# haotiansun14/rl-rep

Measured on NVIDIA B200. Metric: agent updates/sec, higher is better.
Workload: dtype tf32

## Files before the change

include/rlrep_b200.h:

```cpp
#ifndef RLREP_B200_H_
#define RLREP_B200_H_

#include <stddef.h>
#include <stdint.h>

#ifdef __cplusplus
extern "C" {
#endif

#if defined(__GNUC__)
#define RLREP_EXPORT __attribute__((visibility("default")))
#else
#define RLREP_EXPORT
#endif

#define RLREP_ABI_VERSION 3

RLREP_EXPORT int rlrep_abi_version(void);
RLREP_EXPORT const char* rlrep_last_error(void);


enum { RLREP_ACT_NONE = 0, RLREP_ACT_ELU = 1, RLREP_ACT_RELU = 2, RLREP_ACT_TANH = 3, RLREP_ACT_SIN = 4 };
enum {
  RLREP_DACT_NONE = 0,
// ... 185 lines not shown
RLREP_EXPORT int rlrep_mulv_tensor_read(rlrep_mulv* h, int i, float* out_host);
RLREP_EXPORT int rlrep_mulv_tensor_write(rlrep_mulv* h, int i, const float* in_host);
RLREP_EXPORT int rlrep_mulv_sync_targets(rlrep_mulv* h);
RLREP_EXPORT int rlrep_mulv_update(rlrep_mulv* h, const unsigned char* img, const float* action, const float* reward,
                                   const float* discount, const unsigned char* next_img, const unsigned char* img_step1,
                                   const int* shifts, const float* eps_z, const float* eps_act, const float* noise,
                                   float stddev, float* metrics_host);
RLREP_EXPORT int rlrep_mulv_act_batch(rlrep_mulv* h, const unsigned char* obs, const float* eps_host, float stddev, int n,
                                      float* actions_host);
RLREP_EXPORT int rlrep_mulv_act(rlrep_mulv* h, const unsigned char* obs_host, const float* eps_host, float stddev,
                                float* action_host);
RLREP_EXPORT int rlrep_mulv_update_resident(rlrep_mulv* h, int n_steps, float stddev, float* total_ms);
RLREP_EXPORT int rlrep_mulv_profile_update(rlrep_mulv* h, float stddev, int max_entries, const char** names, float* ms,
                                           double* bytes, double* flops, int* n_entries);
RLREP_EXPORT int rlrep_mulv_last_launches(rlrep_mulv* h, int* launches);

typedef struct rlrep_ldiff rlrep_ldiff;
typedef struct rlrep_ldiff_config {
  int batch_size, action_dim, latent_dim, feature_dim, bn_dim, psi_hidden_dim, psi_hidden_depth, zeta_hidden_dim,
      zeta_hidden_depth, hidden_dim;
  double ae_lr, score_lr, actor_lr, critic_lr, weight_decay;
  float tau, kl_coef, ae_coef, stddev_clip;
  int precision;
} rlrep_ldiff_config;
typedef struct rlrep_ldiff_inputs {
  const unsigned char* frames;
  const unsigned char* next_frames;
  const int* shifts;
  const int* next_shifts;
  const float *action, *reward, *discount;
  const float* eps_post;
  const float *alphabar, *temb, *noise;
  const float* psi_masks;
  const float* zeta_masks;
  const float* eps_act;
  float stddev;
} rlrep_ldiff_inputs;
RLREP_EXPORT int rlrep_ldiff_create(const rlrep_ldiff_config* cfg, void* stream, rlrep_ldiff** out);
RLREP_EXPORT int rlrep_ldiff_destroy(rlrep_ldiff* h);
RLREP_EXPORT int rlrep_ldiff_num_tensors(rlrep_ldiff* h, int* n);
RLREP_EXPORT int rlrep_ldiff_tensor_info(rlrep_ldiff* h, int i, const char** name, float** ptr_dev, int* rows, int* cols);
RLREP_EXPORT int rlrep_ldiff_tensor_read(rlrep_ldiff* h, int i, float* out_host);
RLREP_EXPORT int rlrep_ldiff_tensor_write(rlrep_ldiff* h, int i, const float* in_host);
RLREP_EXPORT int rlrep_ldiff_sync_targets(rlrep_ldiff* h);
RLREP_EXPORT int rlrep_ldiff_update(rlrep_ldiff* h, const rlrep_ldiff_inputs* in, float* metrics_host);
RLREP_EXPORT int rlrep_ldiff_update_resident(rlrep_ldiff* h, int n_steps, float stddev, float* total_ms);
RLREP_EXPORT int rlrep_ldiff_profile_update(rlrep_ldiff* h, float stddev, int max_entries, const char** names, float* ms,
                                            double* bytes, double* flops, int* n_entries);
RLREP_EXPORT int rlrep_ldiff_last_launches(rlrep_ldiff* h, int* launches);

RLREP_EXPORT int rlrep_agent_act_batch(rlrep_agent* agent, const float* states_host, const float* eps_host, int rows,
                                       float* actions_host);
RLREP_EXPORT int rlrep_agent_last_launches(rlrep_agent* agent, int* launches);

#ifdef __cplusplus
}
#endif
#endif
```

rlrep_b200/_lib.py:

```python
from __future__ import annotations

import ctypes as C
from pathlib import Path

_HERE = Path(__file__).resolve().parent
LIB_PATH = _HERE / "librlrep_b200.so"


class RlrepError(RuntimeError):
    pass


class OptimState(C.Structure):
    _fields_ = [("steps", C.c_int), ("t_feature", C.c_longlong), ("t_critic", C.c_longlong), ("t_actor", C.c_longlong),
                ("t_alpha", C.c_longlong), ("log_alpha", C.c_double), ("log_alpha_m", C.c_double),
                ("log_alpha_v", C.c_double)]


class AgentConfig(C.Structure):
    _fields_ = [
        ("alg", C.c_int), ("state_dim", C.c_int), ("action_dim", C.c_int), ("batch_size", C.c_int),
        ("hidden_dim", C.c_int), ("feature_dim", C.c_int), ("actor_hidden_dim", C.c_int), ("feature_steps", C.c_int),
        ("lr_critic", C.c_double), ("lr_feature", C.c_double), ("lr_actor", C.c_double), ("lr_alpha", C.c_double),
        ("discount", C.c_float), ("tau", C.c_float), ("feature_tau", C.c_float), ("alpha", C.c_double),
# ... 91 lines not shown
                                     C.POINTER(C.c_double), C.POINTER(i)],
        "rlrep_gemm_set_debug_buffer": [vp],
        "rlrep_ldiff_create": [vp, vp, C.POINTER(vp)],
        "rlrep_ldiff_destroy": [vp],
        "rlrep_ldiff_num_tensors": [vp, C.POINTER(i)],
        "rlrep_ldiff_tensor_info": [vp, i, C.POINTER(C.c_char_p), C.POINTER(vp), C.POINTER(i), C.POINTER(i)],
        "rlrep_ldiff_tensor_read": [vp, i, vp],
        "rlrep_ldiff_tensor_write": [vp, i, vp],
        "rlrep_ldiff_sync_targets": [vp],
        "rlrep_ldiff_update": [vp, vp, vp],
        "rlrep_ldiff_update_resident": [vp, i, C.c_float, C.POINTER(C.c_float)],
        "rlrep_ldiff_profile_update": [vp, C.c_float, i, C.POINTER(C.c_char_p), C.POINTER(C.c_float),
                                       C.POINTER(C.c_double), C.POINTER(C.c_double), C.POINTER(i)],
        "rlrep_ldiff_last_launches": [vp, C.POINTER(i)],
        "rlrep_mulv_create": [vp, vp, C.POINTER(vp)],
        "rlrep_mulv_destroy": [vp],
        "rlrep_mulv_num_tensors": [vp, C.POINTER(i)],
        "rlrep_mulv_tensor_info": [vp, i, C.POINTER(C.c_char_p), C.POINTER(vp), C.POINTER(i), C.POINTER(i)],
        "rlrep_mulv_tensor_read": [vp, i, vp],
        "rlrep_mulv_tensor_write": [vp, i, vp],
        "rlrep_mulv_sync_targets": [vp],
        "rlrep_mulv_update": [vp, vp, vp, vp, vp, vp, vp, vp, vp, vp, vp, C.c_float, vp],
        "rlrep_mulv_last_launches": [vp, C.POINTER(i)],
        "rlrep_mulv_act": [vp, vp, vp, C.c_float, vp],
        "rlrep_mulv_act_batch": [vp, vp, vp, C.c_float, i, vp],
        "rlrep_mulv_update_resident": [vp, i, C.c_float, C.POINTER(C.c_float)],
        "rlrep_mulv_profile_update": [vp, C.c_float, i, C.POINTER(C.c_char_p), C.POINTER(C.c_float), C.POINTER(C.c_double),
                                      C.POINTER(C.c_double), C.POINTER(i)],
        "rlrep_comm_unique_id": [vp],
        "rlrep_comm_create": [vp, i, i, C.POINTER(vp)],
        "rlrep_comm_destroy": [vp],
        "rlrep_comm_info": [vp, C.POINTER(i), C.POINTER(i), C.POINTER(i), C.POINTER(C.c_longlong)],
        "rlrep_agent_create_sharded": [C.POINTER(AgentConfig), vp, vp, C.POINTER(vp)],
        "rlrep_agent_num_tensors": [vp, C.POINTER(i)],
        "rlrep_agent_tensor_info": [vp, i, C.POINTER(C.c_char_p), C.POINTER(vp), C.POINTER(i), C.POINTER(i)],
        "rlrep_agent_tensor_read": [vp, i, vp],
        "rlrep_agent_tensor_write": [vp, i, vp],
        "rlrep_agent_sync_targets": [vp],
        "rlrep_agent_get_log_alpha": [vp, C.POINTER(C.c_double)],
        "rlrep_agent_set_log_alpha": [vp, C.c_double],
        "rlrep_agent_get_steps": [vp, C.POINTER(i)],
        "rlrep_agent_get_optim_state": [vp, C.POINTER(OptimState)],
        "rlrep_agent_set_optim_state": [vp, C.POINTER(OptimState)],
        "rlrep_agent_train_counts": [vp, C.POINTER(i), C.POINTER(i), C.POINTER(i)],
        "rlrep_agent_train": [vp, vp, vp, i, vp, i, vp, i],
        "rlrep_agent_act": [vp, vp, vp, vp],
        "rlrep_pixring_create": [C.c_longlong, i, i, i, i, C.POINTER(vp)],
        "rlrep_pixring_destroy": [vp],
        "rlrep_pixring_write": [vp, C.c_longlong, i, vp, vp, C.c_float, C.c_float, i],
        "rlrep_pixring_flush": [vp],
        "rlrep_pixring_gather": [vp, vp, i, vp, C.c_float, vp, vp, vp, vp, vp, vp],
        "rlrep_agent_act_batch": [vp, vp, vp, i, vp],
        "rlrep_agent_last_launches": [vp, C.POINTER(i)],
        "rlrep_agent_train_resident": [vp, vp, vp, vp, i, C.POINTER(C.c_float)],
        "rlrep_agent_profile_train": [vp, vp, vp, vp, i, C.POINTER(C.c_char_p), C.POINTER(C.c_float),
                                      C.POINTER(C.c_double), C.POINTER(C.c_double), C.POINTER(i)],
    }
    lib.rlrep_agent_metric_name.argtypes = [vp, i]
    lib.rlrep_agent_metric_name.restype = C.c_char_p
    for name, argtypes in sigs.items():
        fn = getattr(lib, name)
        fn.argtypes = argtypes
        fn.restype = C.c_int


def check(rc: int) -> None:
    if rc != 0:
        msg = load().rlrep_last_error()
        raise RlrepError(msg.decode() if msg else f"rlrep call failed with code {rc}")


def current_stream_ptr() -> int:
    import torch
    return torch.cuda.current_stream().cuda_stream


def make_epilogue(bias=None, r1=None, aux=None, pre_out=None, act="none", dact="none", accumulate=False,
                  scale=1.0) -> Epilogue:
    e = Epilogue()
    e.bias = bias.data_ptr() if bias is not None else None
    if r1 is not None:
        e.r1_u, e.r1_v = r1[0].data_ptr(), r1[1].data_ptr()
    if aux is not None:
        e.aux, e.ld_aux = aux.data_ptr(), aux.stride(0)
    if pre_out is not None:
        e.pre_out, e.ld_pre = pre_out.data_ptr(), pre_out.stride(0)
    e.act, e.dact = ACT[act], DACT[dact]
    e.accumulate = int(accumulate)
    e.scale = scale
    return e


def gemm(A, B, C_out, *, a_mn=False, b_mn=False, path="tc", epi: Epilogue | None = None, A2=None, bn=0, split_k=0,
         ws=None):
    lib = load()
    M = A.shape[1] if a_mn else A.shape[0]
    K = A.shape[0] if a_mn else A.shape[1]
    N = B.shape[1] if b_mn else B.shape[0]
    K1 = K
    if A2 is not None:
        K += A2.shape[1]
    assert (B.shape[0] if b_mn else B.shape[1]) == K
    epi = epi or make_epilogue()
    rc = lib.rlrep_gemm(current_stream_ptr(), 0 if path == "tc" else 1, M, N, K, A.data_ptr(), A.stride(0), int(a_mn),
                        A2.data_ptr() if A2 is not None else None, A2.stride(0) if A2 is not None else 0, K1,
                        B.data_ptr(), B.stride(0), int(b_mn), C_out.data_ptr(), C_out.stride(0), C.byref(epi), bn,
# ... 38 lines not shown
```

rlrep_b200/agents.py:

```python
from __future__ import annotations

import ctypes as C
import math

import numpy as np
import torch

from . import _lib


def _orthogonal(out_f, in_f):
    w = torch.empty(out_f, in_f)
    torch.nn.init.orthogonal_(w)
    return w


def _default_linear(out_f, in_f):
    bound = 1.0 / math.sqrt(in_f)
    return (torch.rand(out_f, in_f) * 2 - 1) * bound, (torch.rand(out_f) * 2 - 1) * bound


class _Handle:

    def __init__(self, cfg: _lib.AgentConfig, comm=None):
# ... 52 lines not shown
        i, _, rows, cols = self.index[name]
        lr, lc = self._logical_shape(name, rows, cols)
        arr = torch.as_tensor(value).detach().cpu().float().reshape(-1)
        if arr.numel() != lr * lc:
            raise ValueError(f"{name}: expected {lr * lc} values, got {arr.numel()}")
        if (lr, lc) != (rows, cols):
            full = torch.zeros(rows, cols)
            full[:lr, :lc] = arr.reshape(lr, lc)
            arr = full.reshape(-1)
        arr = np.ascontiguousarray(arr.numpy())
        _lib.check(self.lib.rlrep_agent_tensor_write(self.h, i, arr.ctypes.data))

    def train(self, ring_handle, idx: np.ndarray, eps) -> np.ndarray:
        if isinstance(eps, torch.Tensor):
            torch.cuda.current_stream(eps.device).synchronize()
            eps_ptr, n_eps = eps.data_ptr(), eps.numel()
        else:
            eps_ptr, n_eps = eps.ctypes.data, eps.size
        _lib.check(self.lib.rlrep_agent_train(self.h, ring_handle, idx.ctypes.data, idx.size, eps_ptr, n_eps,
                                              self._metrics.ctypes.data, self._metrics.size))
        return self._metrics

    @property
    def log_alpha(self) -> float:
        v = C.c_double()
        _lib.check(self.lib.rlrep_agent_get_log_alpha(self.h, C.byref(v)))
        return v.value

    @log_alpha.setter
    def log_alpha(self, v):
        _lib.check(self.lib.rlrep_agent_set_log_alpha(self.h, float(v)))

    @property
    def optim_state(self) -> dict:
        st = _lib.OptimState()
        _lib.check(self.lib.rlrep_agent_get_optim_state(self.h, C.byref(st)))
        return {k: getattr(st, k) for k, _ in _lib.OptimState._fields_}

    @optim_state.setter
    def optim_state(self, d):
        st = _lib.OptimState()
        _lib.check(self.lib.rlrep_agent_get_optim_state(self.h, C.byref(st)))
        for k, _ in _lib.OptimState._fields_:
            if k in d:
                setattr(st, k, type(getattr(st, k))(d[k]))
        _lib.check(self.lib.rlrep_agent_set_optim_state(self.h, C.byref(st)))

    @property
    def last_launches(self) -> int:
        v = C.c_int()
        _lib.check(self.lib.rlrep_agent_last_launches(self.h, C.byref(v)))
        return v.value


class SACAgent:

    alg = "sac"

    def __init__(self, state_dim, action_dim, action_space, lr=3e-4, discount=0.99, target_update_period=2, tau=0.005,
                 alpha=0.1, auto_entropy_tuning=True, hidden_dim=1024, *, precision="tf32", use_cuda_graph=True,
                 noise_device="cpu", **extra):
        if noise_device not in ("cpu", "cuda"):
            raise ValueError("noise_device must be 'cpu' or 'cuda'")
        self.noise_device = noise_device
        self.steps = 0
        self.state_dim, self.action_dim = int(state_dim), int(action_dim)
        self.action_range = [float(action_space.low.min()), float(action_space.high.max())]
        self.discount, self.tau = float(discount), float(tau)
        self.target_update_period = int(target_update_period)
        self.learnable_temperature = bool(auto_entropy_tuning)
        self.target_entropy = -action_dim
        self._lr, self._alpha0, self._hidden = float(lr), float(alpha), int(hidden_dim)
        self._precision, self._use_graph = precision, bool(use_cuda_graph)
        self._extra = extra
        self._h: _Handle | None = None
        self._batch = None
        self._pending_state = self._initial_state()

    def _config(self, batch_size) -> _lib.AgentConfig:
        c = _lib.AgentConfig()
        c.alg = _lib.ALG[self.alg]
        c.state_dim, c.action_dim, c.batch_size = self.state_dim, self.action_dim, int(batch_size)
        c.hidden_dim, c.feature_dim, c.actor_hidden_dim = self._pad(self._hidden), 0, self._pad(self._hidden)
        c.feature_steps = 0
        c.lr_critic = c.lr_actor = c.lr_alpha = self._lr
        c.lr_feature = 0.0
        c.discount, c.tau, c.feature_tau = self.discount, self.tau, 0.0
        c.alpha = self._alpha0
        c.target_update_period = self.target_update_period
        c.auto_entropy_tuning = int(self.learnable_temperature)
        c.use_feature_target = 0
        c.precision = _lib.PRECISION[self._precision]
        c.use_cuda_graph = int(self._use_graph)
        return c

    def _layers(self):
        S, A, H = self.state_dim, self.action_dim, self._hidden
        q = [(f"critic.{h}.{i}", o, n, "orth") for h in ("Q1", "Q2") for i, o, n in ((0, H, S + A), (2, H, H), (4, 1, H))]
        return q + self._actor_layers(H)

    def _actor_layers(self, H):
        S, A = self.state_dim, self.action_dim
        return [("actor.trunk.0", H, S, "orth"), ("actor.trunk.2", H, H, "orth"), ("actor.trunk.4", 2 * A, H, "orth")]

    def _initial_state(self):
        sd = {}
# ... 479 lines not shown
```

rlrep_b200/csrc/agent.cuh:

```cuda
#pragma once
#include <cuda_runtime.h>

#include <cstdint>
#include <cstring>
#include <functional>
#include <memory>
#include <string>
#include <unordered_map>
#include <vector>

#include "common.cuh"
#include "gemm.cuh"
#include "gemm_chain.cuh"
#include "kernels.cuh"

namespace rlrep {

class DeviceArena {
 public:
  DeviceArena() = default;
  DeviceArena(const DeviceArena&) = delete;
  DeviceArena& operator=(const DeviceArena&) = delete;
  ~DeviceArena() { release(); }
  template <typename T>
// ... 159 lines not shown
enum Precision : int { PREC_TF32 = 0, PREC_FP32 = 1 };

class GemmRunner {
 public:
  void init(Precision prec, size_t ws_floats);
  ~GemmRunner();
  void run(const GemmArgs& a, cudaStream_t s);
  bool run_compact(GemmArgs a, int wp, int ho, cudaStream_t s);
  bool compact_supported(GemmArgs a, int wp, int ho);
  void set_sm_share(double share) { sm_share_ = share; }

  bool chains_enabled() const { return prec_ == PREC_TF32; }
  void begin_chain(cudaStream_t s);
  void end_chain();
  bool recording() const { return recording_; }

 private:
  void flush_chain();
  bool recording_ = false;
  cudaStream_t chain_stream_ = nullptr;
  std::vector<GemmArgs> pending_;
  std::vector<std::unique_ptr<GemmChain>> chains_;
  Precision prec_ = PREC_TF32;
  double sm_share_ = 1.0;
  float* ws_ = nullptr;
  size_t ws_floats_ = 0;
  float* kg_ws_ = nullptr;
  size_t kg_ws_floats_ = 0;
  std::unordered_map<std::string, TcGemmPlan> plans_;
};

struct Mat {
  const float* p = nullptr;
  int ld = 0;
};
void linear_fwd(GemmRunner& g, cudaStream_t s, int rows, Mat x, const Linear& l, int act, float* y, int ldy,
                Mat x2 = Mat(), int k1 = 0, float* pre_out = nullptr);
void linear_dgrad(GemmRunner& g, cudaStream_t s, int rows, Mat dy, const Linear& l, int dact, Mat aux, float* dx,
                  int lddx, int col0 = 0, int n_cols = -1);
void linear_wgrad(GemmRunner& g, cudaStream_t s, int rows, Mat dy, Mat x, const Linear& l, Mat x2 = Mat(), int k1 = 0,
                  bool bias_grad = true);
inline ColJob bias_job(int rows, Mat dy, const Linear& l) {
  ColJob j;
  j.X = dy.p; j.ld = dy.ld; j.rows = rows; j.cols = l.out; j.u = nullptr; j.out = l.db;
  return j;
}

class GraphReplay {
 public:
  ~GraphReplay() { reset(); }
  void reset();
  void run(cudaStream_t s, bool enabled, const std::function<void()>& body);
  bool captured() const { return exec_ != nullptr; }

 private:
  int calls_ = 0;
  cudaGraph_t graph_ = nullptr;
  cudaGraphExec_t exec_ = nullptr;
};

struct AgentConfig {
  int alg = 0;
  int state_dim = 0, action_dim = 0, batch = 256;
  int hidden_dim = 256, feature_dim = 256, actor_hidden_dim = 256;
  int k_feat = 0;
  double lr = 3e-4, lr_feat = 1e-4, lr_actor = 1e-4, lr_alpha = 1e-4;
  float discount = 0.99f, tau = 0.005f, feature_tau = 0.005f;
  double alpha0 = 0.1;
  int target_update_period = 2, learn_alpha = 1, use_feature_target = 1;
  int precision = PREC_TF32;
  int use_graph = 1;
  int phi_hidden_dim = 0, phi_hidden_depth = 0, mu_hidden_dim = 0, mu_hidden_depth = 0;
  int nabla_hidden_dim = 0, nabla_hidden_depth = 0, num_noise = 20, num_noises = 1000;
  float sigma_scale = 0.449f;
};

class Agent {
 public:
  virtual ~Agent() = default;
  virtual void train(Ring& ring, const long long* idx_host, int n_idx, const float* eps_host, int n_eps,
                     float* metrics_host, int n_metrics) = 0;
  virtual float train_resident(Ring& ring, const long long* idx_host, const float* eps_host, int n_steps) = 0;
  virtual std::vector<ProfileEntry> profile_train(Ring& ring, const long long* idx_host, const float* eps_host) = 0;
  virtual int idx_per_train() const = 0;
  virtual int eps_per_train() const = 0;
  virtual const std::vector<std::string>& metric_names() const = 0;
  virtual std::vector<ParamGroup*> groups() = 0;
  virtual void act(const float* state_host, const float* eps_host, float* action_host) = 0;
  virtual void act_batch(const float* states_host, const float* eps_host, int rows, float* actions_host) = 0;
  virtual void sync_targets_from_params() = 0;

  AgentConfig cfg;
  cudaStream_t stream = nullptr;
  Control* ctl = nullptr;
  int last_launches = 0;
};

std::unique_ptr<Agent> make_sac_agent(const AgentConfig& cfg, cudaStream_t s);
std::unique_ptr<Agent> make_ctrlsac_agent(const AgentConfig& cfg, cudaStream_t s);
std::unique_ptr<Agent> make_vlsac_agent(const AgentConfig& cfg, cudaStream_t s);
std::unique_ptr<Agent> make_spedersac_agent(const AgentConfig& cfg, cudaStream_t s);
std::unique_ptr<Agent> make_diffsrsac_agent(const AgentConfig& cfg, cudaStream_t s);
class Comm;
std::unique_ptr<Agent> make_ctrlsac_sharded_agent(const AgentConfig& cfg, cudaStream_t s, Comm* comm);

}
```

rlrep_b200/csrc/agent_base.cuh:

```cuda
#pragma once
#include "staging.cuh"

#include "agent.cuh"

namespace rlrep {

class SacBase : public Agent {
 public:
  SacBase(const AgentConfig& c, cudaStream_t s) {
    cfg = c;
    stream = s;
    S_ = c.state_dim;
    A_ = c.action_dim;
    B_ = c.batch;
    AH_ = c.actor_hidden_dim;
    RLREP_CHECK(S_ > 0 && A_ > 0 && B_ > 0, "bad agent dimensions");
  }
  ~SacBase() override {
    for (cudaEvent_t e : events_) cudaEventDestroy(e);
    if (side_) cudaStreamDestroy(side_);
    for (cudaStream_t a : aux_)
      if (a) cudaStreamDestroy(a);
    if (metrics_host_) cudaFreeHost(metrics_host_);
    if (idx_host_) cudaFreeHost(idx_host_);
// ... 29 lines not shown
    std::memcpy(metrics_host, metrics_host_, metric_names().size() * sizeof(float));
  }

  float train_resident(Ring& ring, const long long* idx_host, const float* eps_host, int n_steps) override {
    const int ni = idx_per_train(), ne = eps_per_train();
    RLREP_CHECK(ring.S == S_ && ring.A == A_ && n_steps > 0, "bad arguments");
    bind_ring(ring);
    long long* idx_all = nullptr;
    float* eps_all = nullptr;
    RLREP_CUDA(cudaMalloc(&idx_all, (size_t)n_steps * ni * sizeof(long long)));
    RLREP_CUDA(cudaMalloc(&eps_all, (size_t)n_steps * ne * sizeof(float)));
    RLREP_CUDA(cudaMemcpy(idx_all, idx_host, (size_t)n_steps * ni * sizeof(long long), cudaMemcpyHostToDevice));
    RLREP_CUDA(cudaMemcpy(eps_all, eps_host, (size_t)n_steps * ne * sizeof(float), cudaMemcpyHostToDevice));
    cudaEvent_t e0, e1;
    RLREP_CUDA(cudaEventCreate(&e0));
    RLREP_CUDA(cudaEventCreate(&e1));
    RLREP_CUDA(cudaStreamSynchronize(stream));
    RLREP_CUDA(cudaEventRecord(e0, stream));
    for (int i = 0; i < n_steps; ++i) {
      RLREP_CUDA(cudaMemcpyAsync(idx_dev_, idx_all + (size_t)i * ni, (size_t)ni * sizeof(long long),
                                 cudaMemcpyDeviceToDevice, stream));
      RLREP_CUDA(cudaMemcpyAsync(eps_dev_, eps_all + (size_t)i * ne, (size_t)ne * sizeof(float),
                                 cudaMemcpyDeviceToDevice, stream));
      graph_.run(stream, cfg.use_graph != 0, [&] { update(ring); });
    }
    RLREP_CUDA(cudaEventRecord(e1, stream));
    RLREP_CUDA(cudaEventSynchronize(e1));
    float ms = 0.f;
    RLREP_CUDA(cudaEventElapsedTime(&ms, e0, e1));
    cudaEventDestroy(e0);
    cudaEventDestroy(e1);
    cudaFree(idx_all);
    cudaFree(eps_all);
    return ms;
  }

  std::vector<ProfileEntry> profile_train(Ring& ring, const long long* idx_host, const float* eps_host) override {
    const int ni = idx_per_train(), ne = eps_per_train();
    RLREP_CUDA(cudaStreamSynchronize(stream));
    std::memcpy(idx_host_, idx_host, (size_t)ni * sizeof(long long));
    std::memcpy(eps_host_, eps_host, (size_t)ne * sizeof(float));
    RLREP_CUDA(cudaMemcpyAsync(idx_dev_, idx_host_, (size_t)ni * sizeof(long long), cudaMemcpyHostToDevice, stream));
    RLREP_CUDA(cudaMemcpyAsync(eps_dev_, eps_host_, (size_t)ne * sizeof(float), cudaMemcpyHostToDevice, stream));
    serial_ = true;
    profile_begin(stream);
    try {
      update(ring);
    } catch (...) {
      serial_ = false;
      throw;
    }
    serial_ = false;
    return profile_end(stream);
  }

  void act(const float* state_host, const float* eps_host, float* action_host) override {
    act_batch(state_host, eps_host, 1, action_host);
  }
  void act_batch(const float* states_host, const float* eps_host, int rows, float* actions_host) override {
    RLREP_CHECK(rows >= 0 && states_host && actions_host, "bad arguments");
    const Linear l0 = a0_.view(actor_g_), l1 = a1_.view(actor_g_), l2 = a2_.view(actor_g_);
    const int W = S_ + A_;
    for (int done = 0; done < rows; done += kActRows) {
      const int n = std::min(kActRows, rows - done);
      RLREP_CUDA(cudaStreamSynchronize(stream));
      for (int r = 0; r < n; ++r) {
        float* dst = act_in_host_ + (size_t)r * W;
        std::memcpy(dst, states_host + (size_t)(done + r) * S_, S_ * sizeof(float));
        if (eps_host) std::memcpy(dst + S_, eps_host + (size_t)(done + r) * A_, A_ * sizeof(float));
      }
      launch_actor_act(act_in_dev_, n, S_, A_, AH_, l0.W, l0.ld, l0.b, l1.W, l1.ld, l1.b, l2.W, l2.ld, l2.b,
                       eps_host != nullptr, act_out_dev_, stream);
      RLREP_CUDA(cudaStreamSynchronize(stream));
      std::memcpy(actions_host + (size_t)done * A_, act_out_host_, (size_t)n * A_ * sizeof(float));
    }
  }

 protected:
  void bind_ring(const Ring& ring) {
    if (ring_bound_ != ring.generation) {
      graph_.reset();
      ring_bound_ = ring.generation;
    }
  }
  virtual void update(Ring& ring) = 0;

  cudaStream_t side() {
    if (serial_) return stream;
    if (side_ == nullptr) RLREP_CUDA(cudaStreamCreateWithFlags(&side_, cudaStreamNonBlocking));
    return side_;
  }
  cudaEvent_t next_event() {
    if (ev_next_ == events_.size()) {
      cudaEvent_t e;
      RLREP_CUDA(cudaEventCreateWithFlags(&e, cudaEventDisableTiming));
      events_.push_back(e);
    }
    return events_[ev_next_++];
  }
  void fork() {
    gemm_.set_sm_share(dual_share_);
    if (serial_) return;
    cudaEvent_t e = next_event();
    RLREP_CUDA(cudaEventRecord(e, stream));
    RLREP_CUDA(cudaStreamWaitEvent(side(), e, 0));
  }
// ... 48 lines not shown
    arena_.want(&bh2_, (size_t)B_ * AH_);
    arena_.want(&bhead_, (size_t)B_ * round_up32(2 * A_));
    arena_.want(&logp_, B_);
    arena_.want(&dhead_, (size_t)B_ * LDH_);
    arena_.want(&dah2_, (size_t)B_ * AH_);
    arena_.want(&dah1_, (size_t)B_ * AH_);
    LDSA_ = round_up32(S_ + A_);
    arena_.want(&dsa_, (size_t)B_ * LDSA_);
    arena_.want(&cat_next_, (size_t)B_ * LDSA_);
    arena_.want(&cat_pi_, (size_t)B_ * LDSA_);
    arena_.want(&dlogp_, 4);
    RLREP_CUDA(cudaMallocHost(&metrics_host_, kNumMetrics * sizeof(float)));
    RLREP_CUDA(cudaMallocHost(&idx_host_, (size_t)(n_idx > 0 ? n_idx : 1) * sizeof(long long)));
    RLREP_CUDA(cudaMallocHost(&eps_host_, (size_t)(n_eps > 0 ? n_eps : 1) * sizeof(float)));
    RLREP_CUDA(cudaHostAlloc(&act_in_host_, (size_t)kActRows * (S_ + A_) * sizeof(float), cudaHostAllocMapped));
    RLREP_CUDA(cudaHostAlloc(&act_out_host_, (size_t)kActRows * A_ * sizeof(float), cudaHostAllocMapped));
    std::memset(act_in_host_, 0, (size_t)kActRows * (S_ + A_) * sizeof(float));
    RLREP_CUDA(cudaHostGetDevicePointer(&act_in_dev_, act_in_host_, 0));
    RLREP_CUDA(cudaHostGetDevicePointer(&act_out_dev_, act_out_host_, 0));
  }

  void finish_setup(size_t gemm_ws_floats) {
    arena_.commit();
    gemm_.init(static_cast<Precision>(cfg.precision), gemm_ws_floats);
    Control h;
    std::memset(&h, 0, sizeof(h));
    h.log_alpha = std::log(cfg.alpha0);
    h.alpha = (float)cfg.alpha0;
    RLREP_CUDA(cudaMemcpyAsync(ctl, &h, sizeof(h), cudaMemcpyHostToDevice, stream));
    RLREP_CUDA(cudaStreamSynchronize(stream));
  }

  Mat actor_forward_cat(Mat obs, const float* eps, float* cat_buf, float* logp_out, cudaStream_t s = nullptr, int set = 0) {
    if (s == nullptr) s = stream;
    const Linear l0 = a0_.view(actor_g_), l1 = a1_.view(actor_g_), l2 = a2_.view(actor_g_);
    float* h1 = set == 0 ? ah1_ : bh1_;
    float* h2 = set == 0 ? ah2_ : bh2_;
    float* hd = set == 0 ? head_ : bhead_;
    linear_fwd(gemm_, s, B_, obs, l0, ACT_ELU, h1, AH_);
    linear_fwd(gemm_, s, B_, Mat{h1, AH_}, l1, ACT_ELU, h2, AH_);
    linear_fwd(gemm_, s, B_, Mat{h2, AH_}, l2, ACT_NONE, hd, LDH_);
    launch_actor_sample(hd, LDH_, B_, A_, eps, cat_buf + S_, LDSA_, logp_out, s, obs.p, obs.ld, S_);
    return Mat{cat_buf, LDSA_};
  }
  void actor_trunk(Mat obs, int set, cudaStream_t s) {
    const Linear l0 = a0_.view(actor_g_), l1 = a1_.view(actor_g_), l2 = a2_.view(actor_g_);
    float* h1 = set == 0 ? ah1_ : bh1_;
    float* h2 = set == 0 ? ah2_ : bh2_;
    float* hd = set == 0 ? head_ : bhead_;
    linear_fwd(gemm_, s, B_, obs, l0, ACT_ELU, h1, AH_);
    linear_fwd(gemm_, s, B_, Mat{h1, AH_}, l1, ACT_ELU, h2, AH_);
    linear_fwd(gemm_, s, B_, Mat{h2, AH_}, l2, ACT_NONE, hd, LDH_);
  }
  Mat actor_sample_cat(Mat obs, const float* eps, float* cat_buf, float* logp_out, int set, cudaStream_t s) {
    launch_actor_sample(set == 0 ? head_ : bhead_, LDH_, B_, A_, eps, cat_buf + S_, LDSA_, logp_out, s, obs.p, obs.ld, S_);
    return Mat{cat_buf, LDSA_};
  }
  void actor_backward_chained(Mat obs, const float* eps) {
    const Linear l0 = a0_.view(actor_g_), l1 = a1_.view(actor_g_), l2 = a2_.view(actor_g_);
    launch_actor_sample_bwd(head_, LDH_, B_, A_, eps, dsa_ + S_, LDSA_, dlogp_, dhead_, LDH_, stream);
    gemm_.begin_chain(stream);
    linear_wgrad(gemm_, stream, B_, Mat{dhead_, LDH_}, Mat{ah2_, AH_}, l2, Mat(), 0, false);
    linear_dgrad(gemm_, stream, B_, Mat{dhead_, LDH_}, l2, DACT_ELU_OUT, Mat{ah2_, AH_}, dah2_, AH_);
    linear_wgrad(gemm_, stream, B_, Mat{dah2_, AH_}, Mat{ah1_, AH_}, l1, Mat(), 0, false);
    linear_dgrad(gemm_, stream, B_, Mat{dah2_, AH_}, l1, DACT_ELU_OUT, Mat{ah1_, AH_}, dah1_, AH_);
    linear_wgrad(gemm_, stream, B_, Mat{dah1_, AH_}, obs, l0, Mat(), 0, false);
    gemm_.end_chain();
    const ColJob jobs[3] = {bias_job(B_, Mat{dhead_, LDH_}, l2), bias_job(B_, Mat{dah2_, AH_}, l1),
                            bias_job(B_, Mat{dah1_, AH_}, l0)};
    launch_colreduce_multi(jobs, 3, stream);
  }
  struct ActionGradDst {
    float* dx;
    int ld, col0, n_cols;
  };
  ActionGradDst action_grad_dst(const Linear& first) const {
    if (cfg.precision == PREC_TF32 && first.ld == LDSA_ && B_ >= 64) return {dsa_, LDSA_, 0, LDSA_};
    return {dsa_ + S_, LDSA_, S_, A_};
  }
  void dgrad_to_action(Mat dy, const Linear& first) {
    const ActionGradDst d = action_grad_dst(first);
    linear_dgrad(gemm_, stream, B_, dy, first, DACT_NONE, Mat(), d.dx, d.ld, d.col0, d.n_cols);
  }
  void actor_backward(Mat obs, const float* eps) {
    const Linear l0 = a0_.view(actor_g_), l1 = a1_.view(actor_g_), l2 = a2_.view(actor_g_);
    cudaStream_t w = aux(1);
    launch_actor_sample_bwd(head_, LDH_, B_, A_, eps, dsa_ + S_, LDSA_, dlogp_, dhead_, LDH_, stream);
    wait_for(w, mark(stream));
    linear_wgrad(gemm_, w, B_, Mat{dhead_, LDH_}, Mat{ah2_, AH_}, l2, Mat(), 0, false);
    linear_dgrad(gemm_, stream, B_, Mat{dhead_, LDH_}, l2, DACT_ELU_OUT, Mat{ah2_, AH_}, dah2_, AH_);
    wait_for(w, mark(stream));
    linear_wgrad(gemm_, w, B_, Mat{dah2_, AH_}, Mat{ah1_, AH_}, l1, Mat(), 0, false);
    linear_dgrad(gemm_, stream, B_, Mat{dah2_, AH_}, l1, DACT_ELU_OUT, Mat{ah1_, AH_}, dah1_, AH_);
    linear_wgrad(gemm_, stream, B_, Mat{dah1_, AH_}, obs, l0, Mat(), 0, false);
    wait_for(w, mark(stream));
    {
      const ColJob jobs[3] = {bias_job(B_, Mat{dhead_, LDH_}, l2), bias_job(B_, Mat{dah2_, AH_}, l1),
                              bias_job(B_, Mat{dah1_, AH_}, l0)};
      launch_colreduce_multi(jobs, 3, w);
    }
    join_aux(1, stream);
  }
  void actor_adam() {
    launch_adam_polyak(actor_g_.p, actor_g_.g, actor_g_.m, actor_g_.v, actor_g_.n, &ctl->actor, nullptr, 0, 0.f,
                       nullptr, stream);
  }
  TickParams base_tick() const {
    TickParams t;
    t.k_feat = cfg.k_feat;
// ... 39 lines not shown
```

rlrep_b200/csrc/agent_ctrlsac.cu:

```cuda
#include "agent_base.cuh"

namespace rlrep {

namespace {

class CtrlSacAgent final : public SacBase {
 public:
  CtrlSacAgent(const AgentConfig& c, cudaStream_t s) : SacBase(c, s) {
    H_ = c.hidden_dim;
    D_ = c.feature_dim;
    K_ = c.k_feat;
    RLREP_CHECK(K_ >= 1 && K_ <= kMaxFeatureSteps, "extra_feature_steps out of range");
    const RecordLayout probe_layout = RecordLayout::of(S_, A_);
    off_r_ = probe_layout.off_r;
    off_d_ = probe_layout.off_d;
    off_s2_ = probe_layout.off_s2;
    plan_common(K_ * B_, 2 * B_ * A_, probe_layout.R);

    feat_g_.name = "feature";
    p1_ = add_linear(feat_g_, "phi.l1", H_, S_ + A_);
    p2_ = add_linear(feat_g_, "phi.l2", H_, H_);
    p3_ = add_linear(feat_g_, "phi.l3", D_, H_);
    feat_g_.n_target = feat_g_.n;
    feat_g_.target_prefix_from = "phi.";
// ... 161 lines not shown
      GemmArgs a;
      a.M = B_; a.N = D_; a.K = B_;
      a.A = logits_; a.lda = B_; a.a_mn = true;
      a.B = zphi_; a.ldb = D_; a.b_mn = true;
      a.C = dzmu_; a.ldc = D_;
      a.epi.dact = DACT_TANH_OUT; a.epi.aux = zmu_; a.epi.ld_aux = D_;
      gemm_.run(a, s1);
    }
    wait_for(w1, mark(s1));
    gemm_.set_sm_share(wshare);
    linear_wgrad(gemm_, w1, B_, Mat{dzmu_, D_}, Mat{g2_, H_}, n3, Mat(), 0, false);
    gemm_.set_sm_share(share);
    linear_dgrad(gemm_, s1, B_, Mat{dzmu_, D_}, n3, DACT_ELU_OUT, Mat{g2_, H_}, dg2_, H_);
    wait_for(w1, mark(s1));
    gemm_.set_sm_share(wshare);
    linear_wgrad(gemm_, w1, B_, Mat{dg2_, H_}, Mat{g1_, H_}, n2, Mat(), 0, false);
    gemm_.set_sm_share(share);
    linear_dgrad(gemm_, s1, B_, Mat{dg2_, H_}, n2, DACT_ELU_OUT, Mat{g1_, H_}, dg1_, H_);
    linear_wgrad(gemm_, s1, B_, Mat{dg1_, H_}, s2(), n1, Mat(), 0, false);
    wait_for(w1, mark(s1));
    {
      ColJob jobs[3] = {bias_job(B_, Mat{dzmu_, D_}, n3), bias_job(B_, Mat{dg2_, H_}, n2),
                        bias_job(B_, Mat{dg1_, H_}, n1)};
      launch_colreduce_multi(jobs, 3, w1);
    }
    join_aux(0, s0);
    join_aux(1, s0);
    join();
    launch_adam_polyak(feat_g_.p, feat_g_.g, feat_g_.m, feat_g_.v, feat_g_.n, &ctl->feat[k],
                       cfg.use_feature_target ? feat_g_.target : nullptr, feat_g_.n_target, cfg.feature_tau, nullptr,
                       s0);
  }

  void feature_step_chained(int k, Ring& ring) {
    const Linear l1 = p1_.view(feat_g_), l2 = p2_.view(feat_g_), l3 = p3_.view(feat_g_);
    const Linear n1 = m1_.view(feat_g_), n2 = m2_.view(feat_g_), n3 = m3_.view(feat_g_);
    const Linear th = th_.view(feat_g_);
    const float inv_b = 1.f / (float)B_;
    cudaStream_t s0 = stream;
    launch_gather(ring.data, R_ / 4, idx_dev_ + (size_t)k * B_, B_, batch_, s0);
    gemm_.begin_chain(s0);
    phi_forward(s0, sa(), Mat(), 0, zphi_, h1_, h2_);
    linear_fwd(gemm_, s0, B_, s2(), n1, ACT_ELU, g1_, H_);
    linear_fwd(gemm_, s0, B_, Mat{g1_, H_}, n2, ACT_ELU, g2_, H_);
    linear_fwd(gemm_, s0, B_, Mat{g2_, H_}, n3, ACT_TANH, zmu_, D_);
    {
      GemmArgs a;
      a.M = B_; a.N = B_; a.K = D_;
      a.A = zphi_; a.lda = D_;
      a.B = zmu_; a.ldb = D_;
      a.C = logits_; a.ldc = B_;
      gemm_.run(a, s0);
    }
    gemm_.end_chain();
    launch_contrastive_head(logits_, B_, B_, B_, 0, inv_b, zphi_, D_, D_, th.W, th.b, reward(), R_, loss_rows_, rpred_, drp_,
                            metrics_dev_ + 0, head_ctr_, s0);
    gemm_.begin_chain(s0);
    {
      GemmArgs a;
      a.M = B_; a.N = D_; a.K = B_;
      a.A = logits_; a.lda = B_;
      a.B = zmu_; a.ldb = D_; a.b_mn = true;
      a.C = dzphi_; a.ldc = D_;
      a.epi.r1_u = drp_; a.epi.r1_v = th.W;
      gemm_.run(a, s0);
    }
    {
      GemmArgs a;
      a.M = B_; a.N = D_; a.K = B_;
      a.A = logits_; a.lda = B_; a.a_mn = true;
      a.B = zphi_; a.ldb = D_; a.b_mn = true;
      a.C = dzmu_; a.ldc = D_;
      a.epi.dact = DACT_TANH_OUT; a.epi.aux = zmu_; a.epi.ld_aux = D_;
      gemm_.run(a, s0);
    }
    linear_dgrad(gemm_, s0, B_, Mat{dzphi_, D_}, l3, DACT_ELU_OUT, Mat{h2_, H_}, dh2_, H_);
    linear_dgrad(gemm_, s0, B_, Mat{dzmu_, D_}, n3, DACT_ELU_OUT, Mat{g2_, H_}, dg2_, H_);
    linear_wgrad(gemm_, s0, B_, Mat{dzphi_, D_}, Mat{h2_, H_}, l3, Mat(), 0, false);
    linear_wgrad(gemm_, s0, B_, Mat{dzmu_, D_}, Mat{g2_, H_}, n3, Mat(), 0, false);
    linear_dgrad(gemm_, s0, B_, Mat{dh2_, H_}, l2, DACT_ELU_OUT, Mat{h1_, H_}, dh1_, H_);
    linear_dgrad(gemm_, s0, B_, Mat{dg2_, H_}, n2, DACT_ELU_OUT, Mat{g1_, H_}, dg1_, H_);
    linear_wgrad(gemm_, s0, B_, Mat{dh2_, H_}, Mat{h1_, H_}, l2, Mat(), 0, false);
    linear_wgrad(gemm_, s0, B_, Mat{dg2_, H_}, Mat{g1_, H_}, n2, Mat(), 0, false);
    linear_wgrad(gemm_, s0, B_, Mat{dh1_, H_}, sa(), l1, Mat(), 0, false);
    linear_wgrad(gemm_, s0, B_, Mat{dg1_, H_}, s2(), n1, Mat(), 0, false);
    gemm_.end_chain();
    {
      ColJob jobs[8] = {bias_job(B_, Mat{dzphi_, D_}, l3), bias_job(B_, Mat{dh2_, H_}, l2),
                        bias_job(B_, Mat{dh1_, H_}, l1), ColJob{zphi_, drp_, th.dW, D_, B_, D_},
                        ColJob{drp_, nullptr, th.db, 1, B_, 1},
                        bias_job(B_, Mat{dzmu_, D_}, n3), bias_job(B_, Mat{dg2_, H_}, n2),
                        bias_job(B_, Mat{dg1_, H_}, n1)};
      launch_colreduce_multi(jobs, 8, s0);
    }
    launch_adam_polyak(feat_g_.p, feat_g_.g, feat_g_.m, feat_g_.v, feat_g_.n, &ctl->feat[k],
                       cfg.use_feature_target ? feat_g_.target : nullptr, feat_g_.n_target, cfg.feature_tau, nullptr,
                       s0);
  }

  void critic_step_chained() {
    cudaStream_t s0 = stream;
    const float* eps_next = eps_dev_;
    const float* eps_pi = eps_dev_ + (size_t)B_ * A_;
    const Linear l14t = c14_.view(crit_g_, true), l14 = c14_.view(crit_g_), l2 = c2_.view(crit_g_), l5 = c5_.view(crit_g_);
    const Linear l2t = c2_.view(crit_g_, true), l5t = c5_.view(crit_g_, true);
    gemm_.begin_chain(s0);
    actor_trunk(s2(), 1, s0);
    actor_trunk(Mat{batch_, R_}, 0, s0);
    gemm_.end_chain();
    const Mat s2a = actor_sample_cat(s2(), eps_next, cat_next_, logp2_, 1, s0);
    const Mat spi = actor_sample_cat(Mat{batch_, R_}, eps_pi, cat_pi_, logp_, 0, s0);
    gemm_.begin_chain(s0);
    phi_forward(s0, s2a, Mat(), 0, zmu_, h1_, h2_);
    linear_fwd(gemm_, s0, B_, Mat{zmu_, D_}, l14t, ACT_ELU, hid_t_, 2 * H_);
    phi_forward(s0, sa(), Mat(), 0, zphi_, hb1_, hb2_);
    linear_fwd(gemm_, s0, B_, Mat{zphi_, D_}, l14, ACT_ELU, hid_, 2 * H_);
    phi_forward(s0, spi, Mat(), 0, zpi_, hc1_, hc2_);
    gemm_.end_chain();
    {
      CriticHeadArgs a;
      a.hid_t = hid_t_; a.hid = hid_; a.ldh = 2 * H_; a.H = H_; a.B = B_;
      a.w2t = l2t.W; a.b2t = l2t.b; a.w5t = l5t.W; a.b5t = l5t.b;
      a.w2 = l2.W; a.b2 = l2.b; a.w5 = l5.W; a.b5 = l5.b;
      a.reward = reward(); a.done = done(); a.ld_rd = R_;
      a.logp2 = logp2_; a.gamma = cfg.discount; a.c = ctl;
      a.nq1 = nq1_; a.nq2 = nq2_; a.q1 = q1_; a.q2 = q2_; a.dq1 = dq1_; a.dq2 = dq2_;
      a.dhid = dhid_; a.ld_dh = 2 * H_;
      a.metrics = metrics_dev_ + 3;
      a.counter = head_ctr_ + 1;
      launch_critic_td_head(a, s0);
    }
    {
      ColJob jobs[5] = {ColJob{hid_, dq1_, l2.dW, 2 * H_, B_, H_}, ColJob{dq1_, nullptr, l2.db, 1, B_, 1},
                        ColJob{hid_ + H_, dq2_, l5.dW, 2 * H_, B_, H_}, ColJob{dq2_, nullptr, l5.db, 1, B_, 1},
                        bias_job(B_, Mat{dhid_, 2 * H_}, l14)};
      launch_colreduce_multi(jobs, 5, s0);
    }
    linear_wgrad(gemm_, s0, B_, Mat{dhid_, 2 * H_}, Mat{zphi_, D_}, l14, Mat(), 0, false);
    launch_adam_polyak(crit_g_.p, crit_g_.g, crit_g_.m, crit_g_.v, crit_g_.n, &ctl->critic, crit_g_.target,
                       crit_g_.n_target, cfg.tau, &ctl->polyak_critic, s0);
  }

  void actor_step_chained() {
    const float* eps = eps_dev_ + (size_t)B_ * A_;
    const Linear l14 = c14_.view(crit_g_);
    const Linear l1 = p1_.view(feat_g_), l2 = p2_.view(feat_g_), l3 = p3_.view(feat_g_);
    {
      const Linear c2 = c2_.view(crit_g_), c5 = c5_.view(crit_g_);
      linear_fwd(gemm_, stream, B_, Mat{zpi_, D_}, l14, ACT_ELU, hid_, 2 * H_);
      ActorHeadArgs a;
      a.hid = hid_; a.ldh = 2 * H_; a.H = H_; a.B = B_;
      a.w2 = c2.W; a.b2 = c2.b; a.w5 = c5.W; a.b5 = c5.b;
      a.logp = logp_; a.target_entropy = (float)(-A_); a.learn_alpha = cfg.learn_alpha; a.c = ctl;
      a.q1 = q1_; a.q2 = q2_; a.dq1 = dq1_; a.dq2 = dq2_;
      a.dhid = dhid_; a.ld_dh = 2 * H_;
      a.dlogp_scalar = dlogp_;
      a.metrics = metrics_dev_ + 7;
      a.counter = head_ctr_ + 2;
      launch_actor_head(a, stream);
    }
    gemm_.begin_chain(stream);
    linear_dgrad(gemm_, stream, B_, Mat{dhid_, 2 * H_}, l14, DACT_NONE, Mat(), dzphi_, D_);
    linear_dgrad(gemm_, stream, B_, Mat{dzphi_, D_}, l3, DACT_ELU_OUT, Mat{hc2_, H_}, dh2_, H_);
    linear_dgrad(gemm_, stream, B_, Mat{dh2_, H_}, l2, DACT_ELU_OUT, Mat{hc1_, H_}, dh1_, H_);
// ... 86 lines not shown
```

rlrep_b200/csrc/agent_vlsac.cu:

```cuda
#include "agent_base.cuh"

namespace rlrep {

namespace {

constexpr int VH = 256;

class VlSacAgent final : public SacBase {
 public:
  VlSacAgent(const AgentConfig& c, cudaStream_t s) : SacBase(c, s) {
    H_ = c.hidden_dim;
    D_ = c.feature_dim;
    K_ = c.k_feat;
    NN_ = c.num_noise > 0 ? c.num_noise : 20;
    RLREP_CHECK(K_ >= 1 && K_ <= kMaxFeatureSteps, "extra_feature_steps out of range");
    RLREP_CHECK(H_ % 32 == 0 && D_ % 32 == 0, "hidden_dim and feature_dim must be multiples of 32");
    const RecordLayout lay = RecordLayout::of(S_, A_);
    off_r_ = lay.off_r;
    off_d_ = lay.off_d;
    off_s2_ = lay.off_s2;
    plan_common(K_ * B_, K_ * B_ * D_ + 2 * B_ * A_, lay.R);

    feat_g_.name = "feature";
    f1_ = add_linear(feat_g_, "f.l1", VH, S_ + A_);
// ... 213 lines not shown
                       use_target() ? feat_g_.target : nullptr, feat_g_.n_target, cfg.feature_tau, nullptr, s0);
  }

  struct CriticEval {
    int slot;
    const float* head;
    bool target;
  };
  void critic_forward_chained(const CriticEval* ev, int n) {
    cudaStream_t s = stream;
    for (int i = 0; i < n; ++i) launch_noise_expand(ev[i].head, 2 * D_, B_, D_, noise(), NN_, xs_[ev[i].slot], s);
    gemm_.begin_chain(s);
    for (int i = 0; i < n; ++i)
      linear_fwd(gemm_, s, B_ * NN_, Mat{xs_[ev[i].slot], D_}, c14_.view(crit_g_, ev[i].target), ACT_ELU, hid1_[ev[i].slot], 2 * H_);
    gemm_.end_chain();
    for (int i = 0; i < n; ++i) launch_group_mean(hid1_[ev[i].slot], 2 * H_, B_, NN_, 2 * H_, m20_[ev[i].slot], s);
    gemm_.begin_chain(s);
    for (int i = 0; i < n; ++i) {
      const int slot = ev[i].slot;
      linear_fwd(gemm_, s, B_, Mat{m20_[slot], 2 * H_}, c2_.view(crit_g_, ev[i].target), ACT_ELU, hid2_[slot], H_);
      linear_fwd(gemm_, s, B_, Mat{m20_[slot] + H_, 2 * H_}, c5_.view(crit_g_, ev[i].target), ACT_ELU,
                 hid2_[slot] + (size_t)B_ * H_, H_);
    }
    gemm_.end_chain();
    for (int i = 0; i < n; ++i) {
      const Linear l3 = c3_.view(crit_g_, ev[i].target);
      launch_rowdot(hid2_[ev[i].slot], H_, 2 * B_, H_, l3.W, l3.b, q_[ev[i].slot], s);
    }
  }
  void critic_backward_to_hid1_chained(int slot, bool with_wgrad) {
    const Linear l2 = c2_.view(crit_g_), l5 = c5_.view(crit_g_), l3 = c3_.view(crit_g_);
    launch_outer_dact(dq_, l3.W, 2 * B_, H_, hid2_[slot], H_, DACT_ELU_OUT, dhid2_, H_, stream);
    float* dh2a = dhid2_;
    float* dh2b = dhid2_ + (size_t)B_ * H_;
    gemm_.begin_chain(stream);
    linear_dgrad(gemm_, stream, B_, Mat{dh2a, H_}, l2, DACT_NONE, Mat(), dm20_, 2 * H_);
    linear_dgrad(gemm_, stream, B_, Mat{dh2b, H_}, l5, DACT_NONE, Mat(), dm20_ + H_, 2 * H_);
    if (with_wgrad) {
      linear_wgrad(gemm_, stream, B_, Mat{dh2a, H_}, Mat{m20_[slot], 2 * H_}, l2, Mat(), 0, false);
      linear_wgrad(gemm_, stream, B_, Mat{dh2b, H_}, Mat{m20_[slot] + H_, 2 * H_}, l5, Mat(), 0, false);
    }
    gemm_.end_chain();
    launch_group_mean_bwd(dm20_, hid1_[slot], 2 * H_, B_, NN_, 2 * H_, dhid1_, bpart_, stream);
  }

  void critic_step_chained() {
    const float* eps = eps_dev_ + (size_t)K_ * B_ * D_;
    cudaStream_t s0 = stream;
    const bool tgt = use_target();
    gemm_.begin_chain(s0);
    actor_trunk(s2(), 1, s0);
    actor_trunk(Mat{batch_, R_}, 0, s0);
    gemm_.end_chain();
    const Mat s2a = actor_sample_cat(s2(), eps, cat_next_, logp2_, 1, s0);
    const Mat spi = actor_sample_cat(Mat{batch_, R_}, eps + (size_t)B_ * A_, cat_pi_, logp_, 0, s0);
    gemm_.begin_chain(s0);
    prior_forward(s0, tgt, s2a, Mat(), 0, ph1_[0], ph2_[0], phead_[0]);
    prior_forward(s0, tgt, sa(), Mat(), 0, ph1_[1], ph2_[1], phead_[1]);
    prior_forward(s0, tgt, spi, Mat(), 0, ph1_[2], ph2_[2], phead_[2]);
    gemm_.end_chain();
    const CriticEval ev[2] = {{0, phead_[0], true}, {1, phead_[1], false}};
    critic_forward_chained(ev, 2);
    launch_td_critic_loss(reward(), done(), R_, q_[0], q_[0] + B_, logp2_, q_[1], q_[1] + B_, B_, cfg.discount, ctl, dq_,
                          dq_ + B_, metrics_dev_ + 5, s0);
    const Linear l14 = c14_.view(crit_g_), l2 = c2_.view(crit_g_), l5 = c5_.view(crit_g_), l3 = c3_.view(crit_g_);
    critic_backward_to_hid1_chained(1, true);
    linear_wgrad(gemm_, s0, B_ * NN_, Mat{dhid1_, 2 * H_}, Mat{xs_[1], D_}, l14, Mat(), 0, false);
    {
      const ColJob jobs[5] = {ColJob{hid2_[1], dq_, l3.dW, H_, 2 * B_, H_}, ColJob{dq_, nullptr, l3.db, 1, 2 * B_, 1},
                              bias_job(B_, Mat{dhid2_, H_}, l2), bias_job(B_, Mat{dhid2_ + (size_t)B_ * H_, H_}, l5),
                              bias_job(B_, Mat{bpart_, 2 * H_}, l14)};
      launch_colreduce_multi(jobs, 5, s0);
    }
    launch_adam_polyak(crit_g_.p, crit_g_.g, crit_g_.m, crit_g_.v, crit_g_.n, &ctl->critic, crit_g_.target,
                       crit_g_.n_target, cfg.tau, &ctl->polyak_critic, s0);
  }

  void actor_step_chained() {
    const float* eps = eps_dev_ + (size_t)K_ * B_ * D_ + (size_t)B_ * A_;
    const Mat s{batch_, R_};
    const bool tgt = use_target();
    const CriticEval ev[1] = {{0, phead_[2], false}};
    critic_forward_chained(ev, 1);
    launch_actor_alpha_loss(q_[0], q_[0] + B_, logp_, B_, (float)(-A_), cfg.learn_alpha, ctl, dq_, dq_ + B_, dlogp_,
                            metrics_dev_ + 9, stream);
    const Linear l14 = c14_.view(crit_g_);
    const Linear f1 = f1_.view(feat_g_, tgt), f2 = f2_.view(feat_g_, tgt), fh = fh_.view(feat_g_, tgt);
    critic_backward_to_hid1_chained(0, false);
    linear_dgrad(gemm_, stream, B_ * NN_, Mat{dhid1_, 2 * H_}, l14, DACT_NONE, Mat(), dxs_, D_);
    launch_noise_expand_bwd(dxs_, phead_[2], 2 * D_, B_, D_, noise(), NN_, d_head_, stream);
    gemm_.begin_chain(stream);
    linear_dgrad(gemm_, stream, B_, Mat{d_head_, 2 * D_}, fh, DACT_RELU_OUT, Mat{ph2_[2], VH}, dph2_, VH);
    linear_dgrad(gemm_, stream, B_, Mat{dph2_, VH}, f2, DACT_RELU_OUT, Mat{ph1_[2], VH}, dph1_, VH);
    dgrad_to_action(Mat{dph1_, VH}, f1);
    gemm_.end_chain();
    actor_backward_chained(s, eps);
    actor_adam();
  }

  void critic_forward(cudaStream_t s, int slot, const float* head, bool target) {
    const Linear l14 = c14_.view(crit_g_, target), l2 = c2_.view(crit_g_, target), l5 = c5_.view(crit_g_, target);
    const Linear l3 = c3_.view(crit_g_, target);
    launch_noise_expand(head, 2 * D_, B_, D_, noise(), NN_, xs_[slot], s);
    linear_fwd(gemm_, s, B_ * NN_, Mat{xs_[slot], D_}, l14, ACT_ELU, hid1_[slot], 2 * H_);
    launch_group_mean(hid1_[slot], 2 * H_, B_, NN_, 2 * H_, m20_[slot], s);
    linear_fwd(gemm_, s, B_, Mat{m20_[slot], 2 * H_}, l2, ACT_ELU, hid2_[slot], H_);
    linear_fwd(gemm_, s, B_, Mat{m20_[slot] + H_, 2 * H_}, l5, ACT_ELU, hid2_[slot] + (size_t)B_ * H_, H_);
    launch_rowdot(hid2_[slot], H_, 2 * B_, H_, l3.W, l3.b, q_[slot], s);
// ... 91 lines not shown
```

rlrep_b200/csrc/capi.cu:

```cuda
#include <algorithm>
#include <cmath>
#include <memory>
#include <string>
#include <vector>

#include "agent.cuh"
#include "gemm_chain.cuh"
#include "comm.cuh"
#include "common.cuh"
#include "conv.cuh"
#include "deconv.cuh"
#include "drq.cuh"
#include "layout.cuh"
#include "mulv.cuh"
#include "pixel_replay.cuh"
#include "ldiffsr.cuh"
#include "gemm.cuh"
#include "rlrep_b200.h"

namespace rlrep {
namespace {
thread_local std::string g_last_error;
}
void set_last_error(const std::string& msg) { g_last_error = msg; }
// ... 1128 lines not shown
  h.steps = in->steps;
  h.t_feat = in->t_feature; h.t_critic = in->t_critic; h.t_actor = in->t_actor; h.t_alpha = in->t_alpha;
  h.log_alpha = in->log_alpha; h.la_m = in->log_alpha_m; h.la_v = in->log_alpha_v;
  h.alpha = (float)std::exp(in->log_alpha);
  RLREP_CUDA(cudaMemcpyAsync(agent->impl->ctl, &h, sizeof(h), cudaMemcpyHostToDevice, st));
  RLREP_CUDA(cudaStreamSynchronize(st));
  RLREP_API_END
}
int rlrep_agent_get_steps(rlrep_agent* agent, int* steps) {
  RLREP_API_BEGIN_ON(agent)
  Control h;
  RLREP_CUDA(cudaMemcpyAsync(&h, agent->impl->ctl, sizeof(h), cudaMemcpyDeviceToHost, agent->impl->stream));
  RLREP_CUDA(cudaStreamSynchronize(agent->impl->stream));
  *steps = h.steps;
  RLREP_API_END
}
int rlrep_agent_train_counts(rlrep_agent* agent, int* n_idx, int* n_eps, int* n_metrics) {
  RLREP_API_BEGIN_ON(agent)
  *n_idx = agent->impl->idx_per_train();
  *n_eps = agent->impl->eps_per_train();
  *n_metrics = (int)agent->impl->metric_names().size();
  RLREP_API_END
}
const char* rlrep_agent_metric_name(rlrep_agent* agent, int i) {
  const auto& names = agent->impl->metric_names();
  if (i < 0 || i >= (int)names.size()) return nullptr;
  return names[i].c_str();
}
int rlrep_agent_train(rlrep_agent* agent, rlrep_ring* ring, const int64_t* idx_host, int n_idx, const float* eps_host,
                      int n_eps, float* metrics_host, int n_metrics) {
  RLREP_API_BEGIN_ON(agent)
  RLREP_CHECK(agent && ring && idx_host && eps_host && metrics_host, "null argument");
  agent->impl->train(*ring->impl, reinterpret_cast<const long long*>(idx_host), n_idx, eps_host, n_eps, metrics_host,
                     n_metrics);
  RLREP_API_END
}
int rlrep_agent_act(rlrep_agent* agent, const float* state_host, const float* eps_host, float* action_host) {
  RLREP_API_BEGIN_ON(agent)
  agent->impl->act(state_host, eps_host, action_host);
  RLREP_API_END
}
int rlrep_agent_act_batch(rlrep_agent* agent, const float* states_host, const float* eps_host, int rows,
                          float* actions_host) {
  RLREP_API_BEGIN_ON(agent)
  RLREP_CHECK(agent && states_host && actions_host && rows >= 0, "bad arguments");
  agent->impl->act_batch(states_host, eps_host, rows, actions_host);
  RLREP_API_END
}
int rlrep_agent_last_launches(rlrep_agent* agent, int* launches) {
  RLREP_API_BEGIN_ON(agent)
  *launches = agent->impl->last_launches;
  RLREP_API_END
}
int rlrep_agent_train_resident(rlrep_agent* agent, rlrep_ring* ring, const int64_t* idx_host, const float* eps_host,
                               int n_steps, float* total_ms) {
  RLREP_API_BEGIN_ON(agent)
  RLREP_CHECK(agent && ring && idx_host && eps_host && total_ms, "null argument");
  *total_ms = agent->impl->train_resident(*ring->impl, reinterpret_cast<const long long*>(idx_host), eps_host, n_steps);
  RLREP_API_END
}
int rlrep_agent_profile_train(rlrep_agent* agent, rlrep_ring* ring, const int64_t* idx_host, const float* eps_host,
                              int max_entries, const char** names, float* ms, double* bytes, double* flops,
                              int* n_entries) {
  RLREP_API_BEGIN_ON(agent)
  RLREP_CHECK(agent && ring && idx_host && eps_host && n_entries && (max_entries == 0 || (names && ms)), "null argument");
  std::vector<ProfileEntry> prof =
      agent->impl->profile_train(*ring->impl, reinterpret_cast<const long long*>(idx_host), eps_host);
  const int n = (int)std::min<size_t>(prof.size(), (size_t)max_entries);
  for (int i = 0; i < n; ++i) {
    names[i] = prof[i].name;
    ms[i] = prof[i].ms;
    if (bytes) bytes[i] = prof[i].bytes;
    if (flops) flops[i] = prof[i].flops;
  }
  *n_entries = (int)prof.size();
  RLREP_API_END
}
int rlrep_agent_sync_targets(rlrep_agent* agent) {
  RLREP_API_BEGIN_ON(agent)
  agent->impl->sync_targets_from_params();
  RLREP_API_END
}

}
```

rlrep_b200/csrc/common.cuh:

```cuda
#pragma once
#include <cuda.h>
#include <cuda_runtime.h>

#include <cstdio>
#include <stdexcept>
#include <string>
#include <vector>

namespace rlrep {

constexpr int kNumSMs = 148;

struct Error : std::runtime_error {
  using std::runtime_error::runtime_error;
};

void set_last_error(const std::string& msg);
const char* get_last_error();

#define RLREP_CUDA(expr)                                                                              \
  do {                                                                                                \
    cudaError_t _e = (expr);                                                                          \
    if (_e != cudaSuccess) {                                                                          \
      throw ::rlrep::Error(std::string(#expr) + " failed: " + cudaGetErrorString(_e) + " (" __FILE__ \
                           ":" + std::to_string(__LINE__) + ")");                                     \
    }                                                                                                 \
  } while (0)

#define RLREP_CHECK(cond, msg)                                                                           \
  do {                                                                                                   \
    if (!(cond)) {                                                                                       \
      throw ::rlrep::Error(std::string("check failed: " #cond " -- ") + (msg) + " (" __FILE__ ":" +    \
                           std::to_string(__LINE__) + ")");                                              \
    }                                                                                                    \
  } while (0)

void note_launch(const char* name, cudaStream_t stream, double bytes = 0.0, double flops = 0.0);
long long launch_count();
#define RLREP_LAUNCHED(name, stream)          \
  do {                                        \
    RLREP_CUDA(cudaGetLastError());           \
    ::rlrep::note_launch(name, stream);       \
  } while (0)
#define RLREP_LAUNCHED_W(name, stream, bytes, flops)            \
  do {                                                          \
    RLREP_CUDA(cudaGetLastError());                             \
    ::rlrep::note_launch(name, stream, (bytes), (flops));       \
  } while (0)

void profile_begin(cudaStream_t stream);
struct ProfileEntry {
  const char* name;
  float ms;
  double bytes, flops;
};
std::vector<ProfileEntry> profile_end(cudaStream_t stream);

#define RLREP_API_BEGIN try {
#define RLREP_API_END                              \
  return 0;                                        \
  }                                                \
  catch (const std::exception& ex) {               \
    ::rlrep::set_last_error(ex.what());            \
    return 1;                                      \
  }                                                \
  catch (...) {                                    \
    ::rlrep::set_last_error("unknown exception");  \
    return 2;                                      \
  }

inline int ceil_div(int a, int b) { return (a + b - 1) / b; }

}
```

rlrep_b200/csrc/gemm_chain.cu:

```cuda
#include <algorithm>
#include <cmath>
#include <cstdlib>
#include <cstring>

#include "common.cuh"
#include "gemm_chain.cuh"
#include "ptx.cuh"

namespace rlrep {

namespace {

constexpr int kThreads = 320;
constexpr int kEpiWarps = 8;
constexpr int kStages = 6;
constexpr int kCW = 16;
constexpr int kTwPitch = kCW + 4;
constexpr int kMaxBn = 128;
constexpr int kBM = 128, kBK = 32;
constexpr int kABytes = kBM * kBK * 4;
constexpr int kStageBytes = kABytes + kMaxBn * kBK * 4;
constexpr int kTbufFloats = kEpiWarps * 32 * kTwPitch;
constexpr int kSub = 4, kCtrStride = 32;
constexpr int kDbgItems = 16, kDbgEvents = 10;
// ... 130 lines not shown
      if (epi.accumulate) {
        const float4 c0 = __ldcg(cp);
        v[0] += c0.x; v[1] += c0.y; v[2] += c0.z; v[3] += c0.w;
      }
      *cp = make_float4(v[0], v[1], v[2], v[3]);
    }
  }
}

__global__ void __launch_bounds__(kThreads, 1)
gemm_chain_kernel(const ChainGemmDesc* __restrict__ gemms, const ChainTask* __restrict__ tasks,
                  const int* __restrict__ task_begin, unsigned* __restrict__ done, unsigned* __restrict__ exit_ctr,
                  int n_gemms, unsigned long long* __restrict__ dbg) {
  auto stamp = [&](int item, int ev) {
    if (dbg != nullptr && item < kDbgItems) {
      unsigned long long t;
      asm volatile("mov.u64 %0, %%globaltimer;" : "=l"(t)::"memory");
      dbg[((size_t)blockIdx.x * kDbgItems + item) * kDbgEvents + ev] = t;
    }
  };
  if (threadIdx.x == 0) stamp(kDbgItems - 1, 2);
  extern __shared__ uint8_t smem_raw[];
  uint8_t* smem = reinterpret_cast<uint8_t*>((reinterpret_cast<uintptr_t>(smem_raw) + 1023) & ~uintptr_t(1023));
  uint64_t* full_bar = reinterpret_cast<uint64_t*>(smem + kStages * kStageBytes);
  uint64_t* empty_bar = full_bar + 8;
  uint64_t* acc_full = empty_bar + 8;
  uint64_t* acc_empty = acc_full + 2;
  uint32_t* tmem_slot = reinterpret_cast<uint32_t*>(acc_empty + 2);
  volatile unsigned* arrival = reinterpret_cast<volatile unsigned*>(tmem_slot + 1);
  float* tbuf = reinterpret_cast<float*>(smem + kStages * kStageBytes + 256);

  const int warp = threadIdx.x >> 5, lane = threadIdx.x & 31;
  const int t_begin = task_begin[blockIdx.x], t_end = task_begin[blockIdx.x + 1];

  if (threadIdx.x == 0) {
    for (int s = 0; s < kStages; ++s) {
      ptx::mbar_init(&full_bar[s], 1);
      ptx::mbar_init(&empty_bar[s], 1);
    }
    for (int a = 0; a < 2; ++a) {
      ptx::mbar_init(&acc_full[a], 1);
      ptx::mbar_init(&acc_empty[a], kEpiWarps);
    }
    ptx::fence_mbar_init();
  }
  if (warp == 1) {
    ptx::tmem_alloc(tmem_slot, 2 * kMaxBn);
    ptx::tmem_relinquish();
  }
  ptx::tc_fence_before_sync();
  __syncthreads();
  ptx::tc_fence_after_sync();
  const uint32_t tmem_base = *tmem_slot;

  if (warp == 0) {
    if (lane == 0) {
      int it = 0, last_gemm = -1;
      for (int t = t_begin; t < t_end; ++t) {
        const ChainTask tk = tasks[t];
        const ChainGemmDesc* g = gemms + tk.gemm;
        const int n_deps = g->n_deps;
        const int bn = g->bn, a_mn = g->a_mn, b_mn = g->b_mn;
        const int m0 = (tk.tile % g->tiles_m) * kBM, n0 = (tk.tile / g->tiles_m) * bn;
        const int kb0 = tk.split * g->kb_per_split, kb1 = min(g->nkb, kb0 + g->kb_per_split);
        int dep_id[kChainMaxDeps], dep_tiles[kChainMaxDeps];
#pragma unroll
        for (int d = 0; d < kChainMaxDeps; ++d) {
          dep_id[d] = d < n_deps ? g->dep[d] : 0;
          dep_tiles[d] = d < n_deps ? (int)g->dep_target[d] : 0;
        }
        if (tk.gemm != last_gemm) {
          fence_tensormap_acquire(&g->tmA);
          fence_tensormap_acquire(&g->tmB);
          last_gemm = tk.gemm;
        }
        stamp(t - t_begin, 0);
        if (dbg != nullptr && t - t_begin < kDbgItems)
          dbg[((size_t)blockIdx.x * kDbgItems + (t - t_begin)) * kDbgEvents + 8] =
              (unsigned long long)tk.gemm | ((unsigned long long)tk.tile << 16) | ((unsigned long long)tk.split << 40);
#pragma unroll
        for (int d = 0; d < kChainMaxDeps; ++d)
          if (d < n_deps) wait_counter(done, dep_id[d], dep_tiles[d]);
        if (n_deps > 0) {
          fence_acquire_gpu();
          fence_proxy_async_global();
        }
        stamp(t - t_begin, 1);
        const uint32_t tx = kABytes + bn * kBK * 4;
        for (int kb = kb0; kb < kb1; ++kb, ++it) {
          const int s = it % kStages;
          ptx::mbar_wait(&empty_bar[s], ((it / kStages) & 1) ^ 1);
          ptx::mbar_arrive_expect_tx(&full_bar[s], tx);
          uint8_t* a_dst = smem + s * kStageBytes;
          uint8_t* b_dst = a_dst + kABytes;
          const int k0 = kb * kBK;
          if (!a_mn) ptx::tma_load_2d(a_dst, &g->tmA, &full_bar[s], k0, m0);
          else ptx::tma_load_3d(a_dst, &g->tmA, &full_bar[s], 0, k0, m0 / 32);
          if (!b_mn) ptx::tma_load_2d(b_dst, &g->tmB, &full_bar[s], k0, n0);
          else ptx::tma_load_3d(b_dst, &g->tmB, &full_bar[s], 0, k0, n0 / 32);
        }
        stamp(t - t_begin, 2);
      }
    }
  } else if (warp == 1) {
    if (ptx::elect_one()) {
      int it = 0, tc = 0;
// ... 154 lines not shown
              if (s == 0) {
#pragma unroll
                for (int j = 0; j < kCW / 4; ++j) { a[4 * j] = cur[j].x; a[4 * j + 1] = cur[j].y; a[4 * j + 2] = cur[j].z; a[4 * j + 3] = cur[j].w; }
              } else {
#pragma unroll
                for (int j = 0; j < kCW / 4; ++j) { a[4 * j] += cur[j].x; a[4 * j + 1] += cur[j].y; a[4 * j + 2] += cur[j].z; a[4 * j + 3] += cur[j].w; }
              }
            }
          }
#pragma unroll
          for (int j = 0; j < kCW / 4; ++j)
            *reinterpret_cast<float4*>(tw + lane * kTwPitch + 4 * j) = make_float4(a[4 * j], a[4 * j + 1], a[4 * j + 2], a[4 * j + 3]);
          __syncwarp();
          if (fast) {
#define RLREP_CSTORE(A, D) chain_store_rows<A, D>(epi, ops, tw, C, ldc, M, m0 + 32 * q, gn0, lane)
            RLREP_EPILOGUE_SWITCH(epi, RLREP_CSTORE);
#undef RLREP_CSTORE
          } else if (gn0 < N) {
            const int piece = lane & 3, rsub = lane >> 2;
#pragma unroll 1
            for (int r4 = 0; r4 < 4; ++r4) {
              const int r = r4 * 8 + rsub, om = m0 + 32 * q + r;
              if (om >= M) continue;
#pragma unroll 1
              for (int e = 0; e < 4; ++e) {
                const int on = gn0 + 4 * piece + e;
                if (on < N) {
                  float* cp = C + (size_t)om * ldc + on;
                  *cp = chain_epilogue_scalar(epi, tw[r * kTwPitch + 4 * piece + e], om, on, cp);
                }
              }
            }
          }
          __syncwarp();
        }
        if (threadIdx.x == 64) stamp(t - t_begin, 9);
        epilogue_bar();
        if (threadIdx.x == 64) {
          fence_proxy_async_global();
          const int pub = dist ? tk.tile * split_k + tk.split : tk.tile;
          red_release_add(done + ((size_t)tk.gemm * kSub + (pub % kSub)) * kCtrStride, 1u);
          stamp(t - t_begin, 7);
          if (dist) {
            unsigned* ctr = tile_ctr + tk.tile;
            if (atomicAdd(ctr, 1u) == (unsigned)(2 * split_k - 1)) *ctr = 0;
          }
        }
      }
      ptx::tc_fence_before_sync();
      __syncwarp();
      if (lane == 0) ptx::mbar_arrive(&acc_empty[acc]);
    }
  }
  ptx::tc_fence_before_sync();
  __syncthreads();
  if (warp == 1) ptx::tmem_dealloc(tmem_base, 2 * kMaxBn);
  if (threadIdx.x == 0) {
    const unsigned old = atom_add_acq_rel(exit_ctr, 1u);
    if (old == gridDim.x - 1) {
      for (int i = 0; i < n_gemms * kSub; ++i) done[(size_t)i * kCtrStride] = 0;
      *exit_ctr = 0;
      __threadfence();
    }
    stamp(kDbgItems - 1, 3);
  }
}

struct Range {
  uintptr_t lo = 0, hi = 0;
  bool overlaps(const Range& o) const { return lo < o.hi && o.lo < hi && lo != hi && o.lo != o.hi; }
};
Range range_of(const float* p, long long rows, long long ld, long long cols) {
  Range r;
  if (p == nullptr || rows <= 0 || cols <= 0) return r;
  r.lo = reinterpret_cast<uintptr_t>(p);
  r.hi = r.lo + (size_t)((rows - 1) * ld + cols) * sizeof(float);
  return r;
}
struct Footprint {
  std::vector<Range> reads, writes;
};
Footprint footprint(const GemmArgs& a) {
  Footprint f;
  f.reads.push_back(a.a_mn ? range_of(a.A, a.K, a.lda, a.M) : range_of(a.A, a.M, a.lda, a.K));
  f.reads.push_back(a.b_mn ? range_of(a.B, a.K, a.ldb, a.N) : range_of(a.B, a.N, a.ldb, a.K));
  f.reads.push_back(range_of(a.epi.bias, 1, 0, a.N));
  f.reads.push_back(range_of(a.epi.r1_u, 1, 0, a.M));
  f.reads.push_back(range_of(a.epi.r1_v, 1, 0, a.N));
  if (a.epi.dact != DACT_NONE) f.reads.push_back(range_of(a.epi.aux, a.M, a.epi.ld_aux, a.N));
  f.writes.push_back(range_of(a.C, a.M, a.ldc, a.N));
  if (a.epi.accumulate) f.reads.push_back(f.writes.back());
  f.writes.push_back(range_of(a.epi.pre_out, a.M, a.epi.ld_pre, a.N));
  return f;
}
bool conflicts(const Footprint& earlier, const Footprint& later) {
  for (const Range& w : earlier.writes) {
    for (const Range& r : later.reads)
      if (w.overlaps(r)) return true;
    for (const Range& r : later.writes)
      if (w.overlaps(r)) return true;
  }
  for (const Range& w : later.writes)
    for (const Range& r : earlier.reads)
      if (w.overlaps(r)) return true;
  return false;
}
// ... 189 lines not shown
    flops_ += 2.0 * a.M * a.N * a.K;
  }
  std::vector<ChainTask> tasks;
  std::vector<int> begin(n_cta + 1, 0);
  for (int c = 0; c < n_cta; ++c) {
    begin[c] = (int)tasks.size();
    tasks.insert(tasks.end(), per_cta[c].begin(), per_cta[c].end());
  }
  begin[n_cta] = (int)tasks.size();
  grid_ = n_cta;

  auto up = [](size_t x) { return (x + 255) & ~size_t(255); };
  const size_t o_desc = 0;
  const size_t o_tasks = up(o_desc + sizeof(ChainGemmDesc) * n);
  const size_t o_begin = up(o_tasks + sizeof(ChainTask) * tasks.size());
  const size_t o_done = up(o_begin + sizeof(int) * begin.size());
  const size_t o_exit = up(o_done + sizeof(unsigned) * n * kSub * kCtrStride);
  const size_t o_ctr = up(o_exit + sizeof(unsigned));
  const size_t o_ws = up(o_ctr + sizeof(unsigned) * ctr_count);
  const size_t total_bytes = o_ws + sizeof(float) * ws_floats + 256;
  RLREP_CUDA(cudaMalloc(&dev_, total_bytes));
  RLREP_CUDA(cudaMemset(dev_, 0, o_ws));
  char* base = static_cast<char*>(dev_);
  d_gemms_ = reinterpret_cast<ChainGemmDesc*>(base + o_desc);
  d_tasks_ = reinterpret_cast<ChainTask*>(base + o_tasks);
  d_task_begin_ = reinterpret_cast<int*>(base + o_begin);
  d_done_ = reinterpret_cast<unsigned*>(base + o_done);
  d_exit_ = reinterpret_cast<unsigned*>(base + o_exit);
  for (int i = 0; i < n; ++i) {
    descs[i].tile_ctr = reinterpret_cast<unsigned*>(base + o_ctr) + ctr_off[i];
    descs[i].ws = split[i] > 1 ? reinterpret_cast<float*>(base + o_ws) + ws_off[i] : nullptr;
  }
  RLREP_CUDA(cudaMemcpy(d_gemms_, descs.data(), sizeof(ChainGemmDesc) * n, cudaMemcpyHostToDevice));
  RLREP_CUDA(cudaMemcpy(d_tasks_, tasks.data(), sizeof(ChainTask) * tasks.size(), cudaMemcpyHostToDevice));
  RLREP_CUDA(cudaMemcpy(d_task_begin_, begin.data(), sizeof(int) * begin.size(), cudaMemcpyHostToDevice));
  RLREP_CUDA(cudaDeviceSynchronize());
  if (env_int("RLREP_CHAIN_VERBOSE", 0)) {
    std::fprintf(stderr, "rlrep chain: %d GEMMs, %d levels, %zu items, ws %.1f MB\n", n, levels_, tasks.size(),
                 ws_floats * 4 / 1e6);
    for (int i = 0; i < n; ++i)
      std::fprintf(stderr, "  [%d] L%d M=%d N=%d K=%d a_mn=%d b_mn=%d bn=%d split=%d%s share=%d deps=%d\n", i, level[i],
                   seq[i].M, seq[i].N, seq[i].K, (int)seq[i].a_mn, (int)seq[i].b_mn, bn[i], split[i],
                   dist[i] ? " (distributed)" : "", share[i], (int)deps[i].size());
  }
}

void GemmChain::launch(cudaStream_t stream) {
  RLREP_CHECK(dev_ != nullptr, "chain not built");
  cudaLaunchConfig_t cfg = {};
  cfg.gridDim = dim3(grid_);
  cfg.blockDim = dim3(kThreads);
  cfg.dynamicSmemBytes = kSmemBytes;
  cfg.stream = stream;
  cudaLaunchAttribute attr[1];
  attr[0].id = cudaLaunchAttributeCooperative;
  attr[0].val.cooperative = 1;
  cfg.attrs = attr;
  cfg.numAttrs = 1;
  RLREP_CUDA(cudaLaunchKernelEx(&cfg, gemm_chain_kernel, (const ChainGemmDesc*)d_gemms_, (const ChainTask*)d_tasks_,
                                (const int*)d_task_begin_, d_done_, d_exit_, (int)seq_.size(), g_chain_dbg));
  RLREP_LAUNCHED_W("gemm_chain", stream, bytes_, flops_);
}

}
```

rlrep_b200/csrc/gemm_tc_kernel.cuh:

```cuda
#pragma once
#include <algorithm>
#include <cstdint>

#include "common.cuh"
#include "gemm.cuh"
#include "ptx.cuh"

namespace rlrep {
namespace tc {

constexpr int BM = 128;
constexpr int BK = 32;
constexpr int UMMA_K = 8;
constexpr int kThreads = 512;
constexpr int kSmemBudget = 200 * 1024;

__host__ __device__ constexpr int stage_bytes(int bn) { return (BM + bn) * BK * 4; }
__host__ __device__ constexpr int min_stages_fwd(int bn) { return bn >= 256 ? 3 : 2; }
__host__ __device__ constexpr int num_stages(int bn) {
  return kSmemBudget / stage_bytes(bn) > 8 ? 8 : kSmemBudget / stage_bytes(bn);
}
__host__ __device__ constexpr int slots_bytes(int bn) { return BM * (bn + 4) * 4; }
__host__ __device__ constexpr int smem_bytes(int bn, int stages, bool push = false) {
  return stages * stage_bytes(bn) + 1024 + 256 + (push ? slots_bytes(bn) : 0);
// ... 233 lines not shown
  constexpr uint32_t TMEM_COLS = BN < 32 ? 32 : BN;
  constexpr int LDS = BN + 4;
  static_assert(BN == 32 || BN == 64 || BN == 128 || BN == 256, "BN must be a power of two in [32,256]");
  static_assert(min_stages(BN) <= num_stages(BN), "staging tile must fit in the pipeline buffers");

  extern __shared__ uint8_t smem_raw[];
  uint8_t* smem = reinterpret_cast<uint8_t*>((reinterpret_cast<uintptr_t>(smem_raw) + 1023) & ~uintptr_t(1023));
  uint8_t* sA = smem;
  uint8_t* sB = smem + STAGES * A_BYTES;
  uint64_t* full_bar = reinterpret_cast<uint64_t*>(smem + STAGES * (A_BYTES + B_BYTES));
  uint64_t* empty_bar = full_bar + 8;
  uint64_t* accum_bar = empty_bar + 8;
  uint32_t* tmem_slot = reinterpret_cast<uint32_t*>(accum_bar + 1);
  float* stage = reinterpret_cast<float*>(smem);
  float* slots = reinterpret_cast<float*>(smem + STAGES * (A_BYTES + B_BYTES) + 256);

  const int warp = threadIdx.x >> 5;
  const int lane = threadIdx.x & 31;
  if (threadIdx.x == 0) trace(0);
  const int n0 = blockIdx.x * BN;
  const int m0 = blockIdx.y * BM;
  const int splits = gridDim.z / groups;
  if (groups > 1) C += (size_t)(blockIdx.z / splits) * (size_t)(((M + BM - 1) / BM) * BM) * ldc;
  const int nkb_total = (K + BK - 1) / BK;
  const int kb_begin = blockIdx.z * kb_per_split;
  const int kb_end = min(nkb_total, kb_begin + kb_per_split);
  const int nkb = kb_end - kb_begin;

  auto produce = [&](int it) {
    const int s = it % STAGES;
    ptx::mbar_arrive_expect_tx(&full_bar[s], A_BYTES + B_BYTES);
    const int k0 = (kb_begin + it) * BK;
    uint8_t* a_dst = sA + s * A_BYTES;
    uint8_t* b_dst = sB + s * B_BYTES;
    if (!A_MN) {
      const int t = kb_begin + it;
      if (conv_w > 0) ptx::tma_load_2d(a_dst, &tmA, &full_bar[s], 0, m0 + (t / 3) * conv_w + (t % 3));
      else ptx::tma_load_2d(a_dst, &tmA, &full_bar[s], k0, m0);
    } else {
      ptx::tma_load_3d(a_dst, &tmA, &full_bar[s], 0, k0, m0 / 32);
    }
    if (!B_MN) ptx::tma_load_2d(b_dst, &tmB, &full_bar[s], k0, n0);
    else if (conv_w < 0) ptx::tma_load_4d(b_dst, &tmB, &full_bar[s], 0, k0, (n0 / 32) % 8, (n0 / 32) / 8);
    else ptx::tma_load_3d(b_dst, &tmB, &full_bar[s], 0, k0, n0 / 32);
  };
  const int first_round = nkb < 1 ? nkb : 1;
  if (warp == 0 && lane == 0) {
    for (int s = 0; s < STAGES; ++s) {
      ptx::mbar_init(&full_bar[s], 1);
      ptx::mbar_init(&empty_bar[s], 1);
    }
    ptx::mbar_init(accum_bar, 1);
    ptx::fence_mbar_init();
    for (int it = 0; it < first_round; ++it) produce(it);
  }
  if (warp == 2) {
    ptx::tmem_alloc(tmem_slot, TMEM_COLS);
    ptx::tmem_relinquish();
  }
  ptx::tc_fence_before_sync();
  __syncthreads();
  ptx::tc_fence_after_sync();
  const uint32_t tmem_base = *tmem_slot;
  if (threadIdx.x == 0) trace(1);

  if (warp == 0) {
    if (lane == 0) {
      for (int it = first_round; it < nkb; ++it) {
        const int s = it % STAGES;
        const uint32_t ph = (it / STAGES) & 1;
        ptx::mbar_wait(&empty_bar[s], ph ^ 1);
        produce(it);
      }
    }
  } else if (warp == 1) {
    if (ptx::elect_one()) {
      constexpr uint32_t idesc = ptx::make_idesc_tf32(BM, BN, A_MN, B_MN);
      for (int it = 0; it < nkb; ++it) {
        const int s = it % STAGES;
        const uint32_t ph = (it / STAGES) & 1;
        ptx::mbar_wait(&full_bar[s], ph);
        if (it == 0) trace(2);
        ptx::tc_fence_after_sync();
        const uint32_t a_addr = ptx::smem_u32(sA + s * A_BYTES);
        const uint32_t b_addr = ptx::smem_u32(sB + s * B_BYTES);
#pragma unroll
        for (int k = 0; k < BK / UMMA_K; ++k) {
          const uint64_t adesc = A_MN ? ptx::make_smem_desc(a_addr + k * 1024, 4096, 512, 1)
                                      : ptx::make_smem_desc(a_addr + k * UMMA_K * 4, 16, 1024, 2);
          const uint64_t bdesc = B_MN ? ptx::make_smem_desc(b_addr + k * 1024, 4096, 512, 1)
                                      : ptx::make_smem_desc(b_addr + k * UMMA_K * 4, 16, 1024, 2);
          ptx::mma_tf32_ss(tmem_base, adesc, bdesc, idesc, (it > 0 || k > 0) ? 1u : 0u);
        }
        ptx::mma_commit(&empty_bar[s]);
      }
      ptx::mma_commit(accum_bar);
      trace(3);
    }
  } else if (warp < 6) {
    const int q = warp & 3;
    const int r = 32 * q + lane;
    ptx::mbar_wait(accum_bar, 0);
    if (threadIdx.x == 64) trace(4);
    ptx::tc_fence_after_sync();
    if (push) {
      const int rows_per = BM / splits;
      const uint32_t owner = r / rows_per;
      const uint32_t my_rank = ptx::cluster_ctarank();
      const uint32_t dst_row = ptx::smem_u32(slots) + ((my_rank * rows_per + (r - owner * rows_per)) * LDS) * 4;
#pragma unroll 1
      for (int c = 0; c < BN / 32; ++c) {
        uint32_t v[32];
        ptx::tmem_ld_32x32b_x32(tmem_base + (static_cast<uint32_t>(32 * q) << 16) + c * 32, v);
        ptx::tmem_ld_wait();
#pragma unroll
        for (int j = 0; j < 8; ++j)
          ptx::st_dsmem_f4(dst_row + (c * 32 + 4 * j) * 4, owner,
                           make_float4(__uint_as_float(v[4 * j]), __uint_as_float(v[4 * j + 1]),
                                       __uint_as_float(v[4 * j + 2]), __uint_as_float(v[4 * j + 3])));
      }
    } else {
#pragma unroll 1
      for (int c = 0; c < BN / 32; ++c) {
        uint32_t v[32];
        ptx::tmem_ld_32x32b_x32(tmem_base + (static_cast<uint32_t>(32 * q) << 16) + c * 32, v);
        ptx::tmem_ld_wait();
        float4* dst = reinterpret_cast<float4*>(stage + r * LDS + c * 32);
#pragma unroll
        for (int j = 0; j < 8; ++j)
          dst[j] = make_float4(__uint_as_float(v[4 * j]), __uint_as_float(v[4 * j + 1]), __uint_as_float(v[4 * j + 2]),
                               __uint_as_float(v[4 * j + 3]));
      }
    }
    ptx::tc_fence_before_sync();
  }

  if (threadIdx.x == 64) trace(5);
  if (splits > 1) ptx::cluster_sync(); else __syncthreads();
  if (threadIdx.x == 0) trace(6);
  if (warp == 2) ptx::tmem_dealloc(tmem_base, TMEM_COLS);

  {
    TileStore t;
    t.stage_addr = push ? ptx::smem_u32(slots) : ptx::smem_u32(stage);
    t.lds = LDS;
    t.peer_stride = push ? (uint32_t)((BM / splits) * LDS * 4) : 0u;
    t.c4_shift = BN == 32 ? 3 : (BN == 64 ? 4 : (BN == 128 ? 5 : 6));
    t.splits = splits;
    t.rows_per = BM / splits;
    t.row0 = (splits > 1 ? (int)ptx::cluster_ctarank() : 0) * t.rows_per;
    t.row_bias = push ? 0 : t.row0;
    t.m0 = m0; t.n0 = n0; t.M = M; t.N = N;
    t.C = C; t.ldc = ldc;
    const bool arrived = store_tile(t, &epi);
    if (threadIdx.x == 0) trace(7);
    if (splits > 1 && !push) {
      if (!arrived) ptx::cluster_arrive_relaxed();
      ptx::cluster_wait();
    }
  }

  if (threadIdx.x == 64) trace(8);
}

template <int ACT, int DACT>
__device__ __forceinline__ void persist_store_rows(const Epilogue& epi, const float* tw, float* __restrict__ C, int ldc,
                                                   int M, int m_base, int gn0, int lane) {
  const int piece = lane & 7, rsub = lane >> 3;
#pragma unroll
  for (int r4 = 0; r4 < 8; ++r4) {
    const int r = r4 * 4 + rsub;
    const int om = m_base + r, on = gn0 + 4 * piece;
    if (om < M) {
      const float4 a4 = *reinterpret_cast<const float4*>(tw + r * 36 + 4 * piece);
      float* cp = C + (size_t)om * ldc + on;
      const float in[4] = {a4.x, a4.y, a4.z, a4.w};
      float o[4];
#pragma unroll
      for (int e = 0; e < 4; ++e) o[e] = epilogue_apply<ACT, DACT>(epi, in[e], om, on + e, cp + e);
      *reinterpret_cast<float4*>(cp) = make_float4(o[0], o[1], o[2], o[3]);
    }
  }
}

constexpr int kPersistThreads = 192;

template <int BN, bool A_MN, bool B_MN>
__global__ void __launch_bounds__(kPersistThreads, 1)
gemm_tf32_persistent_kernel(const __grid_constant__ CUtensorMap tmA, const __grid_constant__ CUtensorMap tmB,
                            float* __restrict__ C, int ldc, int M, int N, int K, int conv_w, const Epilogue epi,
                            unsigned long long* __restrict__ dbg) {
  constexpr int STAGES = num_stages(BN);
  auto stamp = [&](int role, int tile) {
// ... 401 lines not shown
    if (p.args.b_mn) launch_conv_halo<true>(p, stream);
    else launch_conv_halo<false>(p, stream);
  } else {
    throw Error("the halo convolution kernel exists for BN = 32, K-major A only");
  }
}

template <int BN, bool A_MN, bool B_MN>
void launch_variant_persistent(const TcGemmPlan& p, cudaStream_t stream) {
  auto kern = gemm_tf32_persistent_kernel<BN, A_MN, B_MN>;
  static bool attr_set = false;
  if (!attr_set) {
    RLREP_CUDA(cudaFuncSetAttribute(kern, cudaFuncAttributeMaxDynamicSharedMemorySize, smem_bytes(BN) + 4 * 32 * 36 * 4));
    attr_set = true;
  }
  const GemmArgs& a = p.args;
  RLREP_CHECK(a.compact_wp == 0 && a.conv_ntaps == 0, "compacting stores / tap lists exist on the halo convolution kernel only");
  const int tiles = ceil_div(a.M, BM) * ceil_div(a.N, BN);
  kern<<<std::min(tiles, kNumSMs), kPersistThreads, smem_bytes(BN) + 4 * 32 * 36 * 4, stream>>>(p.tmA, p.tmB, a.C, a.ldc, a.M, a.N, a.K, a.conv_w, a.epi, g_persist_dbg);
  RLREP_LAUNCHED_W("gemm_tf32_persistent", stream,
                   4.0 * ((double)a.M * (a.conv_w > 0 ? 32 : a.K) + (double)a.N * a.K + (double)a.M * a.N),
                   2.0 * a.M * a.N * a.K);
}

template <int BN, bool A_MN, bool B_MN>
void fill_launch_config(cudaLaunchConfig_t& cfg, cudaLaunchAttribute* attr, dim3 grid, int split_k, int stages,
                        bool push, cudaStream_t stream) {
  auto kern = gemm_tf32_kernel<BN, A_MN, B_MN>;
  static bool attr_set = false;
  if (!attr_set) {
    RLREP_CUDA(cudaFuncSetAttribute(kern, cudaFuncAttributeMaxDynamicSharedMemorySize, kMaxSmem));
    attr_set = true;
  }
  cfg = {};
  cfg.gridDim = grid;
  cfg.blockDim = dim3(kThreads);
  cfg.dynamicSmemBytes = smem_bytes(BN, stages, push);
  cfg.stream = stream;
  attr[0].id = cudaLaunchAttributeClusterDimension;
  attr[0].val.clusterDim.x = 1;
  attr[0].val.clusterDim.y = 1;
  attr[0].val.clusterDim.z = split_k;
  cfg.attrs = attr;
  cfg.numAttrs = 1;
}

template <int BN, bool A_MN, bool B_MN>
void launch_variant(const TcGemmPlan& p, cudaStream_t stream) {
  const GemmArgs& a = p.args;
  RLREP_CHECK(a.compact_wp == 0 && a.conv_ntaps == 0, "compacting stores / tap lists exist on the halo convolution kernel only");
  RLREP_CHECK(p.stages >= (p.push ? 2 : min_stages(BN)) && p.stages <= num_stages(BN), "bad pipeline depth");
  RLREP_CHECK(!p.push || (p.split_k > 1 && smem_bytes(BN, p.stages, true) <= kMaxSmem), "bad push-mode plan");
  cudaLaunchConfig_t cfg;
  cudaLaunchAttribute attr[1];
  fill_launch_config<BN, A_MN, B_MN>(cfg, attr, dim3(ceil_div(a.N, BN), ceil_div(a.M, BM), p.split_k * p.k_groups),
                                     p.split_k, p.stages, p.push, stream);
  RLREP_CUDA(cudaLaunchKernelEx(&cfg, gemm_tf32_kernel<BN, A_MN, B_MN>, p.tmA, p.tmB, a.C, a.ldc, a.M, a.N, a.K,
                                p.kb_per_split, p.stages,
                                (p.push ? 1 : 0) | ((p.k_groups - 1) << 8),
                                a.conv_wgrad_hi > 0 ? -1 : a.conv_w, a.epi));
  g_trace_reader = &read_trace_here;
  RLREP_LAUNCHED_W("gemm_tf32", stream,
                   4.0 * ((double)a.M * (a.conv_w > 0 ? 32 : a.K) + (double)(a.conv_wgrad_hi > 0 ? 128 : a.N) * a.K +
                          (double)a.M * a.N),
                   2.0 * a.M * a.N * a.K);
}

template <int BN, bool A_MN, bool B_MN>
int max_clusters_variant(int split_k, int stages, bool push) {
  cudaLaunchConfig_t cfg;
  cudaLaunchAttribute attr[1];
  fill_launch_config<BN, A_MN, B_MN>(cfg, attr, dim3(1, 1, split_k), split_k, stages, push, nullptr);
  int n = 0;
  if (cudaOccupancyMaxActiveClusters(&n, gemm_tf32_kernel<BN, A_MN, B_MN>, &cfg) != cudaSuccess || n <= 0) {
    cudaGetLastError();
    n = kNumSMs / split_k;
  }
  return n;
}

}

#define RLREP_TC_DEFINE(BN, AMN)                                              \
  void launch_tc_##BN##_##AMN(const TcGemmPlan& p, cudaStream_t stream) {     \
    if (p.halo_rows > 0) {                                                    \
      launch_conv_halo_if<BN, AMN>(p, stream);                                \
      return;                                                                 \
    }                                                                         \
    if (p.persistent) {                                                       \
      if (p.args.b_mn) launch_variant_persistent<BN, (AMN) != 0, true>(p, stream);   \
      else launch_variant_persistent<BN, (AMN) != 0, false>(p, stream);       \
      return;                                                                 \
    }                                                                         \
    if (p.args.b_mn) launch_variant<BN, (AMN) != 0, true>(p, stream);         \
    else launch_variant<BN, (AMN) != 0, false>(p, stream);                    \
  }                                                                           \
  int max_clusters_##BN##_##AMN(bool b_mn, int split_k, int stages, bool push) {          \
    return b_mn ? max_clusters_variant<BN, (AMN) != 0, true>(split_k, stages, push)       \
                : max_clusters_variant<BN, (AMN) != 0, false>(split_k, stages, push);     \
  }
#endif

}
}
```

rlrep_b200/csrc/kernels.cu:

```cuda
#include <cmath>

#include "common.cuh"
#include "epilogue.cuh"
#include "kernels.cuh"
#include "reduce.cuh"

namespace rlrep {

namespace {

__device__ __forceinline__ AdamHyper adam_hyper(double lr, long long t) {
  const double bc1 = 1.0 - pow(0.9, (double)t);
  const double bc2 = 1.0 - pow(0.999, (double)t);
  AdamHyper h;
  h.step_size = (float)(lr / bc1);
  h.bc2_sqrt = (float)sqrt(bc2);
  return h;
}

__global__ void tick_kernel(Control* c, const TickParams p) {
  const int lane = threadIdx.x;
  if (blockIdx.x != 0 || lane >= 32) return;
  const long long t_feat = c->t_feat, t_critic = c->t_critic, t_actor = c->t_actor, t_alpha = c->t_alpha;
  const int steps = c->steps + 1;
  const double log_alpha = c->log_alpha;
  __syncwarp();
  const int k = p.k_feat;
  if (lane < k) c->feat[lane] = adam_hyper(p.lr_feat, t_feat + lane + 1);
  if (lane == k && p.critic_steps) c->critic = adam_hyper(p.lr_critic, t_critic + 1);
  if (lane == k + 1) c->actor = adam_hyper(p.lr_actor, t_actor + 1);
  if (lane == k + 2) c->alpha_step_size = p.lr_alpha / (1.0 - pow(0.9, (double)(t_alpha + 1)));
  if (lane == k + 3) c->alpha_bc2_sqrt = sqrt(1.0 - pow(0.999, (double)(t_alpha + 1)));
  if (lane == k + 4) {
    c->alpha = (float)exp(log_alpha);
    c->steps = steps;
    c->polyak_critic = (steps % p.period == 0) ? 1 : 0;
    c->t_feat = t_feat + k;
    if (p.critic_steps) c->t_critic = t_critic + 1;
    c->t_actor = t_actor + 1;
    c->t_alpha = t_alpha + 1;
  }
}

__global__ void gather_kernel(const float4* __restrict__ ring, int rec4, const long long* __restrict__ idx, int B,
                              float4* __restrict__ out) {
  const int total = B * rec4;
  for (int i = blockIdx.x * blockDim.x + threadIdx.x; i < total; i += gridDim.x * blockDim.x) {
    const int b = i / rec4, c = i - b * rec4;
    out[i] = __ldg(ring + (size_t)idx[b] * rec4 + c);
  }
}
__global__ void ring_write_kernel(float4* __restrict__ ring, int rec4, long long capacity, long long start,
                                  const float4* __restrict__ rows, int n) {
  const int total = n * rec4;
  for (int i = blockIdx.x * blockDim.x + threadIdx.x; i < total; i += gridDim.x * blockDim.x) {
    const int b = i / rec4, c = i - b * rec4;
    ring[(size_t)((start + b) % capacity) * rec4 + c] = rows[i];
  }
}

__global__ void __launch_bounds__(256) ce_rows_kernel(float* __restrict__ logits, int ld, int cols, int diag_off,
                                                      float inv_batch, float* __restrict__ loss_rows) {
  __shared__ float scratch[33];
  const int row = blockIdx.x;
  float* l = logits + (size_t)row * ld;
  float mx = -INFINITY;
  for (int j = threadIdx.x; j < cols; j += 256) mx = fmaxf(mx, l[j]);
  mx = block_max<256>(mx, scratch);
  float sum = 0.f;
  for (int j = threadIdx.x; j < cols; j += 256) sum += expf(l[j] - mx);
  sum = block_sum<256>(sum, scratch);
  const float lse = mx + logf(sum);
  const int dj = diag_off + row;
  if (threadIdx.x == 0) loss_rows[row] = lse - l[dj];
  __syncthreads();
  for (int j = threadIdx.x; j < cols; j += 256) {
    const float pr = expf(l[j] - lse);
    l[j] = (pr - (j == dj ? 1.f : 0.f)) * inv_batch;
  }
}

struct RowDotJobs {
  RowDotJob j[2];
};
__global__ void __launch_bounds__(128) rowdot_kernel(const RowDotJobs jobs, int rows) {
  __shared__ float scratch[33];
  const RowDotJob& jb = jobs.j[blockIdx.y];
  const int row = blockIdx.x;
  const float* x = jb.X + (size_t)row * jb.ld;
  const float* w = jb.w;
  const int D = jb.D;
  float acc = 0.f;
  if (((jb.ld | D) & 3) == 0 && ((reinterpret_cast<uintptr_t>(jb.X) | reinterpret_cast<uintptr_t>(w)) & 15) == 0) {
    const float4* x4 = reinterpret_cast<const float4*>(x);
    const float4* w4 = reinterpret_cast<const float4*>(w);
    float a0 = 0.f, a1 = 0.f, a2 = 0.f, a3 = 0.f;
#pragma unroll 4
    for (int j = threadIdx.x; j < D / 4; j += 128) {
// ... 63 lines not shown
    const float4 a = X[i * 8 + c4], b = X[(i + 32) * 8 + c4], c = X[(i + 64) * 8 + c4], d = X[(i + 96) * 8 + c4];
    acc.x += a.x; acc.y += a.y; acc.z += a.z; acc.w += a.w;
    acc.x += b.x; acc.y += b.y; acc.z += b.z; acc.w += b.w;
    acc.x += c.x; acc.y += c.y; acc.z += c.z; acc.w += c.w;
    acc.x += d.x; acc.y += d.y; acc.z += d.z; acc.w += d.w;
  }
  for (; i < r1; i += 32) {
    const float4 a = X[i * 8 + c4];
    acc.x += a.x; acc.y += a.y; acc.z += a.z; acc.w += a.w;
  }
  part[rg][c4] = acc;
  __syncthreads();
  if (threadIdx.x < 8) {
    float4 t = make_float4(0.f, 0.f, 0.f, 0.f);
#pragma unroll 1
    for (int q = 0; q < 32; ++q) {
      const float4 a = part[q][threadIdx.x];
      t.x += a.x; t.y += a.y; t.z += a.z; t.w += a.w;
    }
    reinterpret_cast<float4*>(partial + (long long)blockIdx.y * 32)[threadIdx.x] = t;
  }
}
__global__ void __launch_bounds__(1024) colsum_tall_stage2_kernel(const float* __restrict__ partial, int chunks, int cols,
                                                                  float* __restrict__ out) {
  __shared__ float part[32][33];
  const int tx = threadIdx.x & 31, ty = threadIdx.x >> 5;
  const int j = blockIdx.x * 32 + tx;
  float t0 = 0.f, t1 = 0.f, t2 = 0.f, t3 = 0.f;
  if (j < cols) {
    int c = ty;
    for (; c + 96 < chunks; c += 128) {
      t0 += partial[(long long)c * cols + j];
      t1 += partial[(long long)(c + 32) * cols + j];
      t2 += partial[(long long)(c + 64) * cols + j];
      t3 += partial[(long long)(c + 96) * cols + j];
    }
    for (; c < chunks; c += 32) t0 += partial[(long long)c * cols + j];
  }
  part[ty][tx] = (t0 + t1) + (t2 + t3);
  __syncthreads();
  if (ty == 0 && j < cols) {
    float v = 0.f;
#pragma unroll
    for (int q = 0; q < 32; ++q) v += part[q][tx];
    out[j] = v;
  }
}

struct ColJobs {
  ColJob j[kMaxColJobs];
};
__global__ void __launch_bounds__(1024) colreduce_multi_kernel(const ColJobs jobs) {
  __shared__ float part[32][33];
  const ColJob& jb = jobs.j[blockIdx.y];
  const int tx = threadIdx.x & 31, ty = threadIdx.x >> 5;
  const int j = blockIdx.x * 32 + tx;
  if (blockIdx.x * 32 >= jb.cols) return;
  float acc = 0.f;
  if (j < jb.cols) {
    const float* x = jb.X + j;
    int i = ty;
    for (; i + 7 * 32 < jb.rows; i += 8 * 32) {
      float v[8], w[8];
#pragma unroll
      for (int q = 0; q < 8; ++q) v[q] = x[(size_t)(i + q * 32) * jb.ld];
      if (jb.u) {
#pragma unroll
        for (int q = 0; q < 8; ++q) w[q] = __ldg(jb.u + i + q * 32);
#pragma unroll
        for (int q = 0; q < 8; ++q) acc = fmaf(w[q], v[q], acc);
      } else {
#pragma unroll
        for (int q = 0; q < 8; ++q) acc += v[q];
      }
    }
    for (; i < jb.rows; i += 32) {
      const float v = x[(size_t)i * jb.ld];
      acc = jb.u ? fmaf(__ldg(jb.u + i), v, acc) : acc + v;
    }
  }
  part[ty][tx] = acc;
  __syncthreads();
  if (ty == 0 && j < jb.cols) {
    float t = 0.f;
#pragma unroll
    for (int k = 0; k < 32; ++k) t += part[k][tx];
    jb.out[j] = t;
  }
}

__global__ void outer_dact_kernel(const float* __restrict__ u, const float* __restrict__ w, int rows, int cols,
                                  const float* __restrict__ aux, int ld_aux, int dact, float* __restrict__ out,
                                  int ld_out) {
  const size_t total = (size_t)rows * cols;
  for (size_t i = (size_t)blockIdx.x * blockDim.x + threadIdx.x; i < total; i += (size_t)gridDim.x * blockDim.x) {
    const int r = (int)(i / cols), c = (int)(i - (size_t)r * cols);
    float v = __ldg(u + r) * __ldg(w + c);
    if (dact != DACT_NONE) v *= apply_dact(aux[(size_t)r * ld_aux + c], dact);
    out[(size_t)r * ld_out + c] = v;
  }
}

__global__ void __launch_bounds__(256) feature_loss_finalize_kernel(const float* __restrict__ loss_rows, int rows,
                                                                    const float* __restrict__ pred,
                                                                    const float* __restrict__ reward, int ld_r,
                                                                    float inv_batch, float* __restrict__ dpred,
                                                                    float* __restrict__ metrics) {
  __shared__ float scratch[33];
  float ce = 0.f, se = 0.f;
  for (int i = threadIdx.x; i < rows; i += 256) {
    ce += loss_rows[i];
    const float d = pred[i] - reward[(size_t)i * ld_r];
    se = fmaf(d, d, se);
    dpred[i] = d * inv_batch;
  }
  ce = block_sum<256>(ce, scratch);
  se = block_sum<256>(se, scratch);
  if (threadIdx.x == 0) {
    const float model = ce * inv_batch;
    const float r = 0.5f * (se * inv_batch);
    metrics[0] = model + r;
    metrics[1] = model;
    metrics[2] = r;
  }
}

__global__ void __launch_bounds__(256) contrastive_head_kernel(float* __restrict__ logits, int ld, int cols, int diag_off,
                                                               float inv_batch, const float* __restrict__ z, int ldz, int D,
                                                               const float* __restrict__ theta_w,
                                                               const float* __restrict__ theta_b,
                                                               const float* __restrict__ reward, int ld_r,
                                                               float* __restrict__ loss_rows, float* __restrict__ pred,
                                                               float* __restrict__ dpred, float* __restrict__ metrics,
                                                               unsigned* __restrict__ counter, int rows) {
  __shared__ float scratch[33];
  __shared__ bool last;
  const int row = blockIdx.x;
  float* l = logits + (size_t)row * ld;
  float mx = -INFINITY;
  for (int j = threadIdx.x; j < cols; j += 256) mx = fmaxf(mx, l[j]);
  mx = block_max<256>(mx, scratch);
  float sum = 0.f;
  for (int j = threadIdx.x; j < cols; j += 256) sum += expf(l[j] - mx);
  sum = block_sum<256>(sum, scratch);
  const float lse = mx + logf(sum);
  const int dj = diag_off + row;
  const float loss = lse - l[dj];
  __syncthreads();
  for (int j = threadIdx.x; j < cols; j += 256) {
    const float pr = expf(l[j] - lse);
    l[j] = (pr - (j == dj ? 1.f : 0.f)) * inv_batch;
  }
  const float* x = z + (size_t)row * ldz;
  float acc = 0.f;
  if (((ldz | D) & 3) == 0 && ((reinterpret_cast<uintptr_t>(z) | reinterpret_cast<uintptr_t>(theta_w)) & 15) == 0) {
    const float4* x4 = reinterpret_cast<const float4*>(x);
    const float4* w4 = reinterpret_cast<const float4*>(theta_w);
    float a0 = 0.f, a1 = 0.f, a2 = 0.f, a3 = 0.f;
    for (int j = threadIdx.x; j < D / 4; j += 256) {
      const float4 xv = x4[j];
      const float4 wv = __ldg(w4 + j);
      a0 = fmaf(xv.x, wv.x, a0); a1 = fmaf(xv.y, wv.y, a1); a2 = fmaf(xv.z, wv.z, a2); a3 = fmaf(xv.w, wv.w, a3);
    }
    acc = (a0 + a1) + (a2 + a3);
  } else {
    for (int j = threadIdx.x; j < D; j += 256) acc = fmaf(x[j], __ldg(theta_w + j), acc);
  }
  acc = block_sum<256>(acc, scratch);
  if (threadIdx.x == 0) {
    const float p = acc + __ldg(theta_b);
    loss_rows[row] = loss;
    pred[row] = p;
    dpred[row] = (p - reward[(size_t)row * ld_r]) * inv_batch;
    __threadfence();
    last = atomicAdd(counter, 1u) == (unsigned)(rows - 1);
  }
  __syncthreads();
  if (!last) return;
  __threadfence();
  float ce = 0.f, se = 0.f;
  for (int i = threadIdx.x; i < rows; i += 256) {
    ce += __ldcg(loss_rows + i);
    const float d = __ldcg(pred + i) - reward[(size_t)i * ld_r];
    se = fmaf(d, d, se);
  }
  ce = block_sum<256>(ce, scratch);
  se = block_sum<256>(se, scratch);
  if (threadIdx.x == 0) {
    const float model = ce * inv_batch;
    const float r = 0.5f * (se * inv_batch);
    metrics[0] = model + r;
    metrics[1] = model;
    metrics[2] = r;
    *counter = 0;
  }
}

constexpr float kLogStdMin = -5.f, kLogStdMax = 2.f;

__global__ void actor_sample_kernel(const float* __restrict__ head, int ld_head, int B, int A,
                                    const float* __restrict__ eps, float* __restrict__ action, int lda,
                                    float* __restrict__ logp, const float* __restrict__ obs, int ld_obs, int S) {
  const int b = (blockIdx.x * blockDim.x + threadIdx.x) >> 5, lane = threadIdx.x & 31;
  if (b >= B) return;
  const float* h = head + (size_t)b * ld_head;
  float lp = 0.f;
  for (int j = lane; j < A; j += 32) {
    const float mu = h[j];
    const float ls = kLogStdMin + 0.5f * (kLogStdMax - kLogStdMin) * (tanhf(h[A + j]) + 1.f);
    const float sd = expf(ls);
    const float u = mu + eps[(size_t)b * A + j] * sd;
    const float d = u - mu;
    const float base = -(d * d) / (2.f * sd * sd) - logf(sd) - 0.91893853320467267f;
    const float z = -2.f * u;
    const float sp = z > 20.f ? z : log1pf(expf(z));
    const float ladj = 2.f * (0.69314718055994531f - u - sp);
    lp += -ladj + base;
    action[(size_t)b * lda + j] = tanhf(u);
  }
  lp = warp_sum(lp);
  if (lane == 0) logp[b] = lp;
  if (obs != nullptr) {
    float* dst = action + (size_t)b * lda - S;
    const float* src = obs + (size_t)b * ld_obs;
    for (int j = lane; j < S; j += 32) dst[j] = src[j];
  }
}

__global__ void __launch_bounds__(256) actor_act_kernel(const float* __restrict__ in, int S, int A, int H,
                                                        const float* __restrict__ W0, int ld0, const float* __restrict__ b0,
                                                        const float* __restrict__ W1, int ld1, const float* __restrict__ b1,
                                                        const float* __restrict__ W2, int ld2, const float* __restrict__ b2,
                                                        int explore, float* __restrict__ out) {
  extern __shared__ float sm[];
  float* x = sm;
  float* h1 = x + ((S + 3) & ~3);
  float* h2 = h1 + H;
  float* hd = h2 + H;
  const int row = blockIdx.x, warp = threadIdx.x >> 5, lane = threadIdx.x & 31, nw = blockDim.x >> 5;
  const float* r = in + (size_t)row * (S + A);
  for (int j = threadIdx.x; j < S; j += blockDim.x) x[j] = r[j];
  __syncthreads();
  auto layer = [&](const float* __restrict__ W, int ld, const float* __restrict__ b, const float* src, int n_in, float* dst,
                   int n_out, bool elu) {
    for (int o = warp; o < n_out; o += nw) {
      const float* w = W + (size_t)o * ld;
      float acc = 0.f;
      for (int j = lane; j < n_in; j += 32) acc = fmaf(__ldg(w + j), src[j], acc);
      acc = warp_sum(acc);
      if (lane == 0) {
        const float v = acc + __ldg(b + o);
        dst[o] = elu ? (v > 0.f ? v : expm1f(v)) : v;
      }
    }
    __syncthreads();
  };
  layer(W0, ld0, b0, x, S, h1, H, true);
  layer(W1, ld1, b1, h1, H, h2, H, true);
  layer(W2, ld2, b2, h2, H, hd, 2 * A, false);
  for (int j = threadIdx.x; j < A; j += blockDim.x) {
    float u = hd[j];
    if (explore) {
      const float ls = kLogStdMin + 0.5f * (kLogStdMax - kLogStdMin) * (tanhf(hd[A + j]) + 1.f);
      u += r[S + j] * expf(ls);
    }
    out[(size_t)row * A + j] = tanhf(u);
  }
}

__global__ void actor_sample_bwd_kernel(const float* __restrict__ head, int ld_head, int B, int A,
                                        const float* __restrict__ eps, const float* __restrict__ d_action, int ldd,
                                        const float* __restrict__ dlogp_scalar, float* __restrict__ dhead, int ld_dh) {
  const int i = blockIdx.x * blockDim.x + threadIdx.x;
  if (i >= B * A) return;
  const int b = i / A, j = i - b * A;
  const float* h = head + (size_t)b * ld_head;
  const float glp = *dlogp_scalar;
  const float mu = h[j];
  const float t = tanhf(h[A + j]);
  const float ls = kLogStdMin + 0.5f * (kLogStdMax - kLogStdMin) * (t + 1.f);
  const float sd = expf(ls);
  const float e = eps[i];
  const float a = tanhf(mu + e * sd);
  const float du = d_action[(size_t)b * ldd + j] * (1.f - a * a) + glp * 2.f * a;
  const float dsd = du * e - glp / sd;
  dhead[(size_t)b * ld_dh + j] = du;
  dhead[(size_t)b * ld_dh + A + j] = dsd * sd * (0.5f * (kLogStdMax - kLogStdMin)) * (1.f - t * t);
}

__global__ void __launch_bounds__(256) td_critic_loss_kernel(const float* __restrict__ reward,
                                                             const float* __restrict__ done, int ld_rd,
                                                             const float* __restrict__ nq1,
                                                             const float* __restrict__ nq2,
                                                             const float* __restrict__ logp2,
                                                             const float* __restrict__ q1, const float* __restrict__ q2,
                                                             int B, int norm_B, float gamma,
                                                             const Control* __restrict__ c, float* __restrict__ dq1,
                                                             float* __restrict__ dq2, float* __restrict__ metrics) {
  __shared__ float scratch[33];
  const float alpha = c->alpha;
  const float inv_b = 1.f / (float)norm_B;
  float l1 = 0.f, l2 = 0.f, s1 = 0.f, s2 = 0.f;
  for (int i = threadIdx.x; i < B; i += 256) {
    const float nq = fminf(nq1[i], nq2[i]) - alpha * logp2[i];
    const float y = reward[(size_t)i * ld_rd] + (1.f - done[(size_t)i * ld_rd]) * gamma * nq;
    const float e1 = q1[i] - y, e2 = q2[i] - y;
    l1 = fmaf(e1, e1, l1);
    l2 = fmaf(e2, e2, l2);
    s1 += q1[i];
    s2 += q2[i];
    dq1[i] = 2.f * e1 * inv_b;
    dq2[i] = 2.f * e2 * inv_b;
  }
  l1 = block_sum<256>(l1, scratch);
  l2 = block_sum<256>(l2, scratch);
  s1 = block_sum<256>(s1, scratch);
  s2 = block_sum<256>(s2, scratch);
  if (threadIdx.x == 0) {
    metrics[0] = l1 * inv_b;
    metrics[1] = l2 * inv_b;
    metrics[2] = s1 * inv_b;
    metrics[3] = s2 * inv_b;
  }
}

// ... 18 lines not shown
    dq2[i] = b < a ? g : (a == b ? 0.5f * g : 0.f);
  }
  la = block_sum<256>(la, scratch);
  ent = block_sum<256>(ent, scratch);
  raw = block_sum<256>(raw, scratch);
  if (threadIdx.x == 0) {
    *dlogp_scalar = alpha * inv_b;
    metrics[0] = la * inv_b;
    const float alpha_loss = ent * inv_b;
    metrics[1] = alpha_loss;
    if (learn_alpha) {
      const double g = (double)(raw * inv_b) * exp(c->log_alpha);
      c->la_m = c->la_m + (1.0 - 0.9) * (g - c->la_m);
      c->la_v = c->la_v * 0.999 + (1.0 - 0.999) * g * g;
      const double denom = sqrt(c->la_v) / c->alpha_bc2_sqrt + 1e-8;
      c->log_alpha = c->log_alpha - c->alpha_step_size * (c->la_m / denom);
    }
    metrics[2] = (float)exp(c->log_alpha);
  }
}

__device__ __forceinline__ float head_dot(const float* __restrict__ x, const float* __restrict__ w, int D, int tid) {
  float acc = 0.f;
  if ((D & 3) == 0 && ((reinterpret_cast<uintptr_t>(x) | reinterpret_cast<uintptr_t>(w)) & 15) == 0) {
    const float4* x4 = reinterpret_cast<const float4*>(x);
    const float4* w4 = reinterpret_cast<const float4*>(w);
    float a0 = 0.f, a1 = 0.f, a2 = 0.f, a3 = 0.f;
    for (int j = tid; j < D / 4; j += 256) {
      const float4 xv = x4[j];
      const float4 wv = __ldg(w4 + j);
      a0 = fmaf(xv.x, wv.x, a0); a1 = fmaf(xv.y, wv.y, a1); a2 = fmaf(xv.z, wv.z, a2); a3 = fmaf(xv.w, wv.w, a3);
    }
    acc = (a0 + a1) + (a2 + a3);
  } else {
    for (int j = tid; j < D; j += 256) acc = fmaf(x[j], __ldg(w + j), acc);
  }
  return acc;
}
__device__ __forceinline__ void head_backward_row(const float* __restrict__ hid, const float* __restrict__ w2,
                                                  const float* __restrict__ w5, float dq1, float dq2, int H,
                                                  float* __restrict__ dhid, int tid) {
  for (int j = tid; j < 2 * H; j += 256) {
    const bool second = j >= H;
    float v = (second ? dq2 : dq1) * __ldg((second ? w5 : w2) + (second ? j - H : j));
    v *= apply_dact(hid[j], DACT_ELU_OUT);
    dhid[j] = v;
  }
}

__global__ void __launch_bounds__(256) critic_td_head_kernel(const CriticHeadArgs a) {
  __shared__ float scratch[33];
  __shared__ float bc[2];
  __shared__ bool last;
  const int row = blockIdx.x, tid = threadIdx.x, H = a.H;
  const float* ht = a.hid_t + (size_t)row * a.ldh;
  const float* h = a.hid + (size_t)row * a.ldh;
  float nq1 = block_sum<256>(head_dot(ht, a.w2t, H, tid), scratch);
  float nq2 = block_sum<256>(head_dot(ht + H, a.w5t, H, tid), scratch);
  float q1 = block_sum<256>(head_dot(h, a.w2, H, tid), scratch);
  float q2 = block_sum<256>(head_dot(h + H, a.w5, H, tid), scratch);
  if (tid == 0) {
    nq1 += __ldg(a.b2t); nq2 += __ldg(a.b5t); q1 += __ldg(a.b2); q2 += __ldg(a.b5);
    const float alpha = a.c->alpha, inv_b = 1.f / (float)a.B;
    const float nq = fminf(nq1, nq2) - alpha * a.logp2[row];
    const float y = a.reward[(size_t)row * a.ld_rd] + (1.f - a.done[(size_t)row * a.ld_rd]) * a.gamma * nq;
    const float e1 = q1 - y, e2 = q2 - y;
    a.nq1[row] = nq1; a.nq2[row] = nq2; a.q1[row] = q1; a.q2[row] = q2;
    bc[0] = 2.f * e1 * inv_b;
    bc[1] = 2.f * e2 * inv_b;
    a.dq1[row] = bc[0];
    a.dq2[row] = bc[1];
  }
  __syncthreads();
  head_backward_row(h, a.w2, a.w5, bc[0], bc[1], H, a.dhid + (size_t)row * a.ld_dh, tid);
  if (tid == 0) {
    __threadfence();
    last = atomicAdd(a.counter, 1u) == (unsigned)(a.B - 1);
  }
  __syncthreads();
  if (!last) return;
  __threadfence();
  const float alpha = a.c->alpha, inv_b = 1.f / (float)a.B;
  float l1 = 0.f, l2 = 0.f, s1 = 0.f, s2 = 0.f;
  for (int i = tid; i < a.B; i += 256) {
    const float nq = fminf(__ldcg(a.nq1 + i), __ldcg(a.nq2 + i)) - alpha * a.logp2[i];
    const float y = a.reward[(size_t)i * a.ld_rd] + (1.f - a.done[(size_t)i * a.ld_rd]) * a.gamma * nq;
    const float v1 = __ldcg(a.q1 + i), v2 = __ldcg(a.q2 + i);
    const float e1 = v1 - y, e2 = v2 - y;
    l1 = fmaf(e1, e1, l1);
    l2 = fmaf(e2, e2, l2);
    s1 += v1;
    s2 += v2;
  }
  l1 = block_sum<256>(l1, scratch);
  l2 = block_sum<256>(l2, scratch);
  s1 = block_sum<256>(s1, scratch);
  s2 = block_sum<256>(s2, scratch);
  if (tid == 0) {
    a.metrics[0] = l1 * inv_b;
    a.metrics[1] = l2 * inv_b;
    a.metrics[2] = s1 * inv_b;
    a.metrics[3] = s2 * inv_b;
    *a.counter = 0;
  }
}

__global__ void __launch_bounds__(256) actor_head_kernel(const ActorHeadArgs a) {
  __shared__ float scratch[33];
  __shared__ float bc[2];
  __shared__ bool last;
  const int row = blockIdx.x, tid = threadIdx.x, H = a.H;
  const float* h = a.hid + (size_t)row * a.ldh;
  float q1 = block_sum<256>(head_dot(h, a.w2, H, tid), scratch);
  float q2 = block_sum<256>(head_dot(h + H, a.w5, H, tid), scratch);
  if (tid == 0) {
    q1 += __ldg(a.b2); q2 += __ldg(a.b5);
    a.q1[row] = q1; a.q2[row] = q2;
    const float g = -1.f / (float)a.B;
    bc[0] = q1 < q2 ? g : (q1 == q2 ? 0.5f * g : 0.f);
    bc[1] = q2 < q1 ? g : (q1 == q2 ? 0.5f * g : 0.f);
    a.dq1[row] = bc[0];
    a.dq2[row] = bc[1];
  }
  __syncthreads();
  head_backward_row(h, a.w2, a.w5, bc[0], bc[1], H, a.dhid + (size_t)row * a.ld_dh, tid);
  if (tid == 0) {
    __threadfence();
    last = atomicAdd(a.counter, 1u) == (unsigned)(a.B - 1);
  }
  __syncthreads();
  if (!last) return;
  __threadfence();
  Control* c = a.c;
  const float alpha = c->alpha, inv_b = 1.f / (float)a.B;
  float la = 0.f, ent = 0.f, raw = 0.f;
  for (int i = tid; i < a.B; i += 256) {
    const float v1 = __ldcg(a.q1 + i), v2 = __ldcg(a.q2 + i);
    la += alpha * a.logp[i] - fminf(v1, v2);
    ent += alpha * (-a.logp[i] - a.target_entropy);
    raw += -a.logp[i] - a.target_entropy;
  }
  la = block_sum<256>(la, scratch);
  ent = block_sum<256>(ent, scratch);
  raw = block_sum<256>(raw, scratch);
  if (tid == 0) {
    *a.dlogp_scalar = alpha * inv_b;
    a.metrics[0] = la * inv_b;
    a.metrics[1] = ent * inv_b;
    if (a.learn_alpha) {
      const double g = (double)(raw * inv_b) * exp(c->log_alpha);
      c->la_m = c->la_m + (1.0 - 0.9) * (g - c->la_m);
      c->la_v = c->la_v * 0.999 + (1.0 - 0.999) * g * g;
      const double denom = sqrt(c->la_v) / c->alpha_bc2_sqrt + 1e-8;
      c->log_alpha = c->log_alpha - c->alpha_step_size * (c->la_m / denom);
    }
    a.metrics[2] = (float)exp(c->log_alpha);
    *a.counter = 0;
  }
}

__global__ void __launch_bounds__(256) actor_loss_partial_kernel(const float* __restrict__ q1,
                                                                 const float* __restrict__ q2,
                                                                 const float* __restrict__ logp, int B, int norm_B,
// ... 4 lines not shown
  __shared__ float scratch[33];
  const float alpha = c->alpha;
  const float inv_b = 1.f / (float)norm_B;
  float la = 0.f, raw = 0.f;
  for (int i = threadIdx.x; i < B; i += 256) {
    const float a = q1[i], b = q2[i];
    la += alpha * logp[i] - fminf(a, b);
    raw += -logp[i] - target_entropy;
    const float g = -inv_b;
    dq1[i] = a < b ? g : (a == b ? 0.5f * g : 0.f);
    dq2[i] = b < a ? g : (a == b ? 0.5f * g : 0.f);
  }
  la = block_sum<256>(la, scratch);
  raw = block_sum<256>(raw, scratch);
  if (threadIdx.x == 0) {
    *dlogp_scalar = alpha * inv_b;
    partial[0] = la * inv_b;
    partial[1] = raw * inv_b;
  }
}
__global__ void alpha_step_kernel(const float* __restrict__ reduced, int learn_alpha, Control* c,
                                  float* __restrict__ metrics) {
  if (threadIdx.x != 0 || blockIdx.x != 0) return;
  metrics[0] = reduced[0];
  metrics[1] = c->alpha * reduced[1];
  if (learn_alpha) {
    const double g = (double)reduced[1] * exp(c->log_alpha);
    c->la_m = c->la_m + (1.0 - 0.9) * (g - c->la_m);
    c->la_v = c->la_v * 0.999 + (1.0 - 0.999) * g * g;
    const double denom = sqrt(c->la_v) / c->alpha_bc2_sqrt + 1e-8;
    c->log_alpha = c->log_alpha - c->alpha_step_size * (c->la_m / denom);
  }
  metrics[2] = (float)exp(c->log_alpha);
}
__global__ void mul_dact_kernel(float* __restrict__ x, const float* __restrict__ aux, size_t n, int dact) {
  for (size_t i = (size_t)blockIdx.x * blockDim.x + threadIdx.x; i < n; i += (size_t)gridDim.x * blockDim.x)
    x[i] *= apply_dact(aux[i], dact);
}

__device__ __forceinline__ float adam_elem(float& p, float g, float& m, float& v, float ss, float bc2s) {
  constexpr float w1 = (float)(1.0 - 0.9), b2 = 0.999f, w2 = (float)(1.0 - 0.999), eps = 1e-8f;
  m = fmaf(w1, g - m, m);
  v = fmaf(w2 * g, g, v * b2);
  const float denom = sqrtf(v) / bc2s + eps;
  p = p - ss * (m / denom);
  return p;
}

__global__ void __launch_bounds__(256) adam_polyak_kernel(float4* __restrict__ p, const float4* __restrict__ g,
                                                          float4* __restrict__ m, float4* __restrict__ v, size_t n4,
                                                          const AdamHyper* __restrict__ hyper,
                                                          float4* __restrict__ target, size_t n4_polyak, float tau,
                                                          const int* __restrict__ polyak_flag) {
  const float ss = hyper->step_size, bc2s = hyper->bc2_sqrt;
  const bool do_polyak = target != nullptr && (polyak_flag == nullptr || *polyak_flag != 0);
  const float omt = 1.f - tau;
  for (size_t i = (size_t)blockIdx.x * blockDim.x + threadIdx.x; i < n4; i += (size_t)gridDim.x * blockDim.x) {
    float4 pv = p[i], mv = __ldcs(m + i), vv = __ldcs(v + i);
    const float4 gv = __ldcs(g + i);
    adam_elem(pv.x, gv.x, mv.x, vv.x, ss, bc2s);
    adam_elem(pv.y, gv.y, mv.y, vv.y, ss, bc2s);
    adam_elem(pv.z, gv.z, mv.z, vv.z, ss, bc2s);
    adam_elem(pv.w, gv.w, mv.w, vv.w, ss, bc2s);
    p[i] = pv;
    __stcs(m + i, mv);
    __stcs(v + i, vv);
    if (do_polyak && i < n4_polyak) {
      float4 t = __ldcs(target + i);
      t.x = __fadd_rn(__fmul_rn(tau, pv.x), __fmul_rn(omt, t.x));
      t.y = __fadd_rn(__fmul_rn(tau, pv.y), __fmul_rn(omt, t.y));
      t.z = __fadd_rn(__fmul_rn(tau, pv.z), __fmul_rn(omt, t.z));
      t.w = __fadd_rn(__fmul_rn(tau, pv.w), __fmul_rn(omt, t.w));
      __stcs(target + i, t);
    }
  }
}

__global__ void __launch_bounds__(256) polyak_kernel(const float4* __restrict__ p, float4* __restrict__ target,
                                                     size_t n4, float tau, const int* __restrict__ polyak_flag) {
  if (polyak_flag != nullptr && *polyak_flag == 0) return;
  const float omt = 1.f - tau;
  for (size_t i = (size_t)blockIdx.x * blockDim.x + threadIdx.x; i < n4; i += (size_t)gridDim.x * blockDim.x) {
    const float4 pv = p[i];
    float4 t = target[i];
    t.x = __fadd_rn(__fmul_rn(tau, pv.x), __fmul_rn(omt, t.x));
    t.y = __fadd_rn(__fmul_rn(tau, pv.y), __fmul_rn(omt, t.y));
    t.z = __fadd_rn(__fmul_rn(tau, pv.z), __fmul_rn(omt, t.z));
    t.w = __fadd_rn(__fmul_rn(tau, pv.w), __fmul_rn(omt, t.w));
    target[i] = t;
  }
}

constexpr float kLogSigMin = -20.f, kLogSigMax = 2.f;
__device__ __forceinline__ float clamp_ls(float raw) { return fminf(fmaxf(raw, kLogSigMin), kLogSigMax); }
__device__ __forceinline__ float clamp_grad(float raw) { return (raw >= kLogSigMin && raw <= kLogSigMax) ? 1.f : 0.f; }

struct ColSegments {
  ColSegment s[3];
  int n;
};
__global__ void pack_columns_kernel(const float* __restrict__ in, int ld_in, float* __restrict__ out, int ld_out, int rows,
                                    const ColSegments segs, int width) {
  const size_t total = (size_t)rows * width;
  for (size_t i = (size_t)blockIdx.x * blockDim.x + threadIdx.x; i < total; i += (size_t)gridDim.x * blockDim.x) {
    const int r = (int)(i / width);
    int c = (int)(i - (size_t)r * width);
// ... 150 lines not shown
__global__ void group_mean_kernel(const float* __restrict__ hid, int ld, int B, int NN, int C, float* __restrict__ out) {
  const int total = B * C;
  const float inv = 1.f / (float)NN;
  for (int i = blockIdx.x * blockDim.x + threadIdx.x; i < total; i += gridDim.x * blockDim.x) {
    const int b = i / C, c = i - b * C;
    float acc = 0.f;
    for (int j = 0; j < NN; ++j) acc += hid[((size_t)b * NN + j) * ld + c];
    out[i] = acc * inv;
  }
}

__global__ void group_mean_bwd_kernel(const float* __restrict__ dmean, const float* __restrict__ hid, int ld, int B, int NN,
                                      int C, float* __restrict__ dhid, float* __restrict__ colsum_partial) {
  const int total = B * C;
  const float inv = 1.f / (float)NN;
  for (int i = blockIdx.x * blockDim.x + threadIdx.x; i < total; i += gridDim.x * blockDim.x) {
    const int b = i / C, c = i - b * C;
    const float g = dmean[i] * inv;
    float acc = 0.f;
    for (int j = 0; j < NN; ++j) {
      const size_t o = ((size_t)b * NN + j) * ld + c;
      const float v = g * apply_dact(hid[o], DACT_ELU_OUT);
      dhid[o] = v;
      acc += v;
    }
    colsum_partial[i] = acc;
  }
}

__global__ void kgroup_finish_kernel(const float* __restrict__ ws, int groups, int M, int N, int ldw, size_t group_stride,
                                     float* __restrict__ C, int ldc, const Epilogue epi) {
  const size_t total = (size_t)M * N;
  for (size_t i = (size_t)blockIdx.x * blockDim.x + threadIdx.x; i < total; i += (size_t)gridDim.x * blockDim.x) {
    const int m = (int)(i / N), n = (int)(i - (size_t)m * N);
    float acc = 0.f;
    for (int g = 0; g < groups; ++g) acc += ws[(size_t)g * group_stride + (size_t)m * ldw + n];
    float* cp = C + (size_t)m * ldc + n;
    *cp = epilogue_apply<-1, -1>(epi, acc, m, n, cp);
  }
}

int grid_for(size_t work_items, int threads, int per_sm = 8) {
  size_t blocks = (work_items + threads - 1) / threads;
  const size_t cap = (size_t)kNumSMs * per_sm;
  if (blocks > cap) blocks = cap;
  if (blocks < 1) blocks = 1;
  return (int)blocks;
}

}

void launch_tick(Control* c, const TickParams& p, cudaStream_t s) {
  RLREP_CHECK(p.k_feat <= kMaxFeatureSteps, "too many feature steps per update");
  tick_kernel<<<1, 32, 0, s>>>(c, p);
  RLREP_LAUNCHED("tick", s);
}

void launch_gather(const float* ring, int rec4, const long long* idx, int B, float* out, cudaStream_t s) {
  gather_kernel<<<grid_for((size_t)B * rec4, 256), 256, 0, s>>>(reinterpret_cast<const float4*>(ring), rec4, idx, B,
                                                               reinterpret_cast<float4*>(out));
  RLREP_LAUNCHED_W("gather", s, 2.0 * 16.0 * (double)B * rec4, 0.0);
}

void launch_ring_write(float* ring, int rec4, long long capacity, long long start, const float* rows, int n,
                       cudaStream_t s) {
  if (n <= 0) return;
  ring_write_kernel<<<grid_for((size_t)n * rec4, 256), 256, 0, s>>>(reinterpret_cast<float4*>(ring), rec4, capacity,
                                                                   start, reinterpret_cast<const float4*>(rows), n);
  RLREP_LAUNCHED("ring_write", s);
}

void launch_ce_rows(float* logits, int ld, int rows, int cols, int diag_off, float inv_batch, float* loss_rows,
                    cudaStream_t s) {
  ce_rows_kernel<<<rows, 256, 0, s>>>(logits, ld, cols, diag_off, inv_batch, loss_rows);
  RLREP_LAUNCHED_W("ce_rows", s, 3.0 * 4.0 * (double)rows * cols, 0.0);
}

void launch_rowdot(const float* X, int ld, int rows, int D, const float* w, const float* b, float* y, cudaStream_t s) {
  RowDotJobs js;
  js.j[0] = RowDotJob{X, w, b, y, ld, D};
  js.j[1] = js.j[0];
  rowdot_kernel<<<dim3(rows, 1), 128, 0, s>>>(js, rows);
  RLREP_LAUNCHED("rowdot", s);
}
void launch_rowdot_pair(const RowDotJob& a, const RowDotJob& b, int rows, cudaStream_t s) {
  RowDotJobs js;
  js.j[0] = a;
  js.j[1] = b;
  rowdot_kernel<<<dim3(rows, 2), 128, 0, s>>>(js, rows);
  RLREP_LAUNCHED("rowdot", s);
}

void launch_colreduce(const float* X, int ld, int rows, int cols, const float* u, float* out, int accumulate,
                      cudaStream_t s) {
  colreduce_kernel<<<ceil_div(cols, 32), 256, 0, s>>>(X, ld, rows, cols, u, out, accumulate);
  RLREP_LAUNCHED("colreduce", s);
}

void launch_colsum_tall(const float* X, int ld, long long rows, int cols, float* partial, int chunks, float* out,
                        cudaStream_t s) {
  const int rows_per = (int)((rows + chunks - 1) / chunks);
  if (cols == 32 && ld == 32 && (reinterpret_cast<uintptr_t>(X) & 15) == 0 && (reinterpret_cast<uintptr_t>(partial) & 15) == 0)
    colsum_tall32_stage1_kernel<<<dim3(1, chunks), 256, 0, s>>>(reinterpret_cast<const float4*>(X), rows, rows_per, partial);
  else
    colsum_tall_stage1_kernel<<<dim3(ceil_div(cols, 32), chunks), 256, 0, s>>>(X, ld, rows, cols, rows_per, partial);
  RLREP_LAUNCHED_W("colsum_tall", s, 4.0 * (double)rows * cols, 0.0);
  colsum_tall_stage2_kernel<<<ceil_div(cols, 32), 1024, 0, s>>>(partial, chunks, cols, out);
  RLREP_LAUNCHED("colsum_tall_final", s);
}

void launch_kgroup_finish(const float* ws, int groups, int M, int N, int ldw, size_t group_stride, float* C, int ldc,
                          const Epilogue& epi, cudaStream_t s) {
  const size_t total = (size_t)M * N;
  kgroup_finish_kernel<<<grid_for(total, 256, 16), 256, 0, s>>>(ws, groups, M, N, ldw, group_stride, C, ldc, epi);
  RLREP_LAUNCHED_W("kgroup_finish", s, 4.0 * (double)total * (groups + 1), 0.0);
}

void launch_colsum_finish(const float* partial, int chunks, int cols, float* out, cudaStream_t s) {
  colsum_tall_stage2_kernel<<<ceil_div(cols, 32), 1024, 0, s>>>(partial, chunks, cols, out);
  RLREP_LAUNCHED("colsum_tall_final", s);
}

void launch_colreduce_multi(const ColJob* jobs, int n_jobs, cudaStream_t s) {
  RLREP_CHECK(n_jobs >= 1 && n_jobs <= kMaxColJobs, "too many column-reduction jobs for one launch");
  ColJobs js;
  int max_cols = 0;
  for (int i = 0; i < n_jobs; ++i) {
    js.j[i] = jobs[i];
    if (jobs[i].cols > max_cols) max_cols = jobs[i].cols;
  }
  colreduce_multi_kernel<<<dim3(ceil_div(max_cols, 32), n_jobs), 1024, 0, s>>>(js);
  RLREP_LAUNCHED("colreduce_multi", s);
}

void launch_outer_dact(const float* u, const float* w, int rows, int cols, const float* aux, int ld_aux, int dact,
                       float* out, int ld_out, cudaStream_t s) {
  outer_dact_kernel<<<grid_for((size_t)rows * cols, 256), 256, 0, s>>>(u, w, rows, cols, aux, ld_aux, dact, out,
                                                                      ld_out);
  RLREP_LAUNCHED("outer_dact", s);
}

void launch_feature_loss_finalize(const float* loss_rows, int rows, const float* pred, const float* reward, int ld_r,
                                  float inv_batch, float* dpred, float* metrics, cudaStream_t s) {
  feature_loss_finalize_kernel<<<1, 256, 0, s>>>(loss_rows, rows, pred, reward, ld_r, inv_batch, dpred, metrics);
  RLREP_LAUNCHED("feature_loss_finalize", s);
}

void launch_contrastive_head(float* logits, int ld, int rows, int cols, int diag_off, float inv_batch, const float* z, int ldz,
                             int D, const float* theta_w, const float* theta_b, const float* reward, int ld_r,
                             float* loss_rows, float* pred, float* dpred, float* metrics, unsigned* counter,
                             cudaStream_t s) {
  contrastive_head_kernel<<<rows, 256, 0, s>>>(logits, ld, cols, diag_off, inv_batch, z, ldz, D, theta_w, theta_b, reward, ld_r,
                                               loss_rows, pred, dpred, metrics, counter, rows);
  RLREP_LAUNCHED_W("contrastive_head", s, 3.0 * 4.0 * (double)rows * cols + 4.0 * (double)rows * D, 0.0);
}

void launch_critic_td_head(const CriticHeadArgs& a, cudaStream_t s) {
  critic_td_head_kernel<<<a.B, 256, 0, s>>>(a);
  RLREP_LAUNCHED_W("critic_td_head", s, 4.0 * a.B * (4.0 * a.H + 2.0 * a.H), 0.0);
}
void launch_actor_head(const ActorHeadArgs& a, cudaStream_t s) {
  actor_head_kernel<<<a.B, 256, 0, s>>>(a);
  RLREP_LAUNCHED_W("actor_head", s, 4.0 * a.B * (4.0 * a.H), 0.0);
}

void launch_actor_sample(const float* head, int ld_head, int B, int A, const float* eps, float* action, int lda,
                         float* logp, cudaStream_t s, const float* obs, int ld_obs, int S) {
  actor_sample_kernel<<<ceil_div(B * 32, 128), 128, 0, s>>>(head, ld_head, B, A, eps, action, lda, logp, obs, ld_obs, S);
  RLREP_LAUNCHED("actor_sample", s);
}

void launch_actor_act(const float* in, int rows, int S, int A, int H, const float* W0, int ld0, const float* b0,
                      const float* W1, int ld1, const float* b1, const float* W2, int ld2, const float* b2, int explore,
                      float* out, cudaStream_t s) {
  const size_t smem = (size_t)(((S + 3) & ~3) + 2 * H + 2 * A) * sizeof(float);
  RLREP_CHECK(smem <= 48 * 1024, "actor too wide for the one-launch select_action kernel");
  actor_act_kernel<<<rows, 256, smem, s>>>(in, S, A, H, W0, ld0, b0, W1, ld1, b1, W2, ld2, b2, explore, out);
  RLREP_LAUNCHED("actor_act", s);
}

void launch_actor_sample_bwd(const float* head, int ld_head, int B, int A, const float* eps, const float* d_action,
                             int ldd, const float* dlogp_scalar, float* dhead, int ld_dhead, cudaStream_t s) {
  actor_sample_bwd_kernel<<<ceil_div(B * A, 128), 128, 0, s>>>(head, ld_head, B, A, eps, d_action, ldd, dlogp_scalar,
                                                               dhead, ld_dhead);
  RLREP_LAUNCHED("actor_sample_bwd", s);
}

void launch_td_critic_loss(const float* reward, const float* done, int ld_rd, const float* nq1, const float* nq2,
                           const float* logp2, const float* q1, const float* q2, int B, float gamma, const Control* c,
                           float* dq1, float* dq2, float* metrics, cudaStream_t s, int norm_B) {
  td_critic_loss_kernel<<<1, 256, 0, s>>>(reward, done, ld_rd, nq1, nq2, logp2, q1, q2, B, norm_B > 0 ? norm_B : B, gamma,
                                          c, dq1, dq2, metrics);
  RLREP_LAUNCHED("td_critic_loss", s);
}

void launch_actor_alpha_loss(const float* q1, const float* q2, const float* logp, int B, float target_entropy,
                             int learn_alpha, Control* c, float* dq1, float* dq2, float* dlogp_scalar, float* metrics,
                             cudaStream_t s) {
  actor_alpha_loss_kernel<<<1, 256, 0, s>>>(q1, q2, logp, B, target_entropy, learn_alpha, c, dq1, dq2, dlogp_scalar,
                                            metrics);
  RLREP_LAUNCHED("actor_alpha_loss", s);
}

void launch_actor_loss_partial(const float* q1, const float* q2, const float* logp, int B, int norm_B,
                               float target_entropy, const Control* c, float* dq1, float* dq2, float* dlogp_scalar,
                               float* partial, cudaStream_t s) {
  actor_loss_partial_kernel<<<1, 256, 0, s>>>(q1, q2, logp, B, norm_B, target_entropy, c, dq1, dq2, dlogp_scalar, partial);
  RLREP_LAUNCHED("actor_loss_partial", s);
}
void launch_alpha_step(const float* reduced, int learn_alpha, Control* c, float* metrics, cudaStream_t s) {
  alpha_step_kernel<<<1, 32, 0, s>>>(reduced, learn_alpha, c, metrics);
  RLREP_LAUNCHED("alpha_step", s);
}
void launch_mul_dact(float* x, const float* aux, size_t n, int dact, cudaStream_t s) {
  mul_dact_kernel<<<grid_for(n, 256), 256, 0, s>>>(x, aux, n, dact);
  RLREP_LAUNCHED_W("mul_dact", s, 12.0 * (double)n, 0.0);
}

void launch_pack_columns(const float* in, int ld_in, float* out, int ld_out, int rows, const ColSegment* segs, int n_segs,
                         cudaStream_t s) {
  RLREP_CHECK(n_segs >= 1 && n_segs <= 3, "pack_columns takes 1..3 segments");
  ColSegments cs;
  cs.n = n_segs;
  int width = 0;
  for (int i = 0; i < n_segs; ++i) {
    cs.s[i] = segs[i];
    width += segs[i].len;
  }
  pack_columns_kernel<<<grid_for((size_t)rows * width, 256), 256, 0, s>>>(in, ld_in, out, ld_out, rows, cs, width);
  RLREP_LAUNCHED("pack_columns", s);
}
void launch_vae_sample(const float* head, int ld_head, int B, int D, const float* eps, float* z, cudaStream_t s) {
  vae_sample_kernel<<<grid_for((size_t)B * D, 256), 256, 0, s>>>(head, ld_head, B, D, eps, z);
  RLREP_LAUNCHED("vae_sample", s);
}
void launch_vae_recon_loss(const float* xr, int ld_xr, const float* next_state, const float* reward, int ld_rec, int B,
                           int S, float* dxr, float* partial, int n_blocks, cudaStream_t s) {
  vae_recon_loss_kernel<<<n_blocks, 256, 0, s>>>(xr, ld_xr, next_state, reward, ld_rec, B, S, dxr, partial);
  RLREP_LAUNCHED("vae_recon_loss", s);
}
void launch_vae_kl_bwd(const float* enc_head, const float* prior_head, int ld_head, int B, int D, const float* eps,
                       const float* dz, float* d_enc, float* d_prior, float* partial, int n_blocks, cudaStream_t s) {
  vae_kl_bwd_kernel<<<n_blocks, 256, 0, s>>>(enc_head, prior_head, ld_head, B, D, eps, dz, d_enc, d_prior, partial);
  RLREP_LAUNCHED("vae_kl_bwd", s);
}
void launch_vae_finalize(const float* recon_partial, int n_recon, const float* kl_partial, int n_kl, int B, int S, int D,
                         float* metrics, cudaStream_t s) {
  vae_finalize_kernel<<<1, 32, 0, s>>>(recon_partial, n_recon, kl_partial, n_kl, B, S, D, metrics);
  RLREP_LAUNCHED("vae_finalize", s);
}
void launch_noise_expand(const float* head, int ld_head, int B, int D, const float* noise, int NN, float* x,
                         cudaStream_t s) {
  const bool vec = (D & 3) == 0 && (ld_head & 3) == 0 && (long long)B * NN * D < (1LL << 31) &&
                   ((reinterpret_cast<uintptr_t>(head) | reinterpret_cast<uintptr_t>(noise) | reinterpret_cast<uintptr_t>(x)) & 15) == 0;
  if (vec) noise_expand4_kernel<<<grid_for((size_t)B * (D / 4), 256, 16), 256, 0, s>>>(head, ld_head, B, D, noise, NN, x);
  else noise_expand_kernel<<<grid_for((size_t)B * NN * D, 256, 16), 256, 0, s>>>(head, ld_head, B, D, noise, NN, x);
  RLREP_LAUNCHED("noise_expand", s);
}
void launch_noise_expand_bwd(const float* dx, const float* head, int ld_head, int B, int D, const float* noise, int NN,
                             float* d_head, cudaStream_t s) {
  noise_expand_bwd_kernel<<<grid_for((size_t)B * D, 256), 256, 0, s>>>(dx, head, ld_head, B, D, noise, NN, d_head);
  RLREP_LAUNCHED("noise_expand_bwd", s);
}
void launch_group_mean(const float* hid, int ld, int B, int NN, int C, float* out, cudaStream_t s) {
  group_mean_kernel<<<grid_for((size_t)B * C, 256), 256, 0, s>>>(hid, ld, B, NN, C, out);
  RLREP_LAUNCHED("group_mean", s);
}
void launch_group_mean_bwd(const float* dmean, const float* hid, int ld, int B, int NN, int C, float* dhid,
                           float* colsum_partial, cudaStream_t s) {
  group_mean_bwd_kernel<<<grid_for((size_t)B * C, 256), 256, 0, s>>>(dmean, hid, ld, B, NN, C, dhid, colsum_partial);
  RLREP_LAUNCHED("group_mean_bwd", s);
}

void launch_adam_polyak(float* p, const float* g, float* m, float* v, size_t n, const AdamHyper* hyper, float* target,
                        size_t n_polyak, float tau, const int* polyak_flag, cudaStream_t s) {
  RLREP_CHECK(n % 4 == 0 && n_polyak % 4 == 0, "optimizer arenas are padded to float4");
  const size_t n4 = n / 4;
  adam_polyak_kernel<<<grid_for(n4, 256, 16), 256, 0, s>>>(
      reinterpret_cast<float4*>(p), reinterpret_cast<const float4*>(g), reinterpret_cast<float4*>(m),
      reinterpret_cast<float4*>(v), n4, hyper, reinterpret_cast<float4*>(target), n_polyak / 4, tau, polyak_flag);
  const double polyak = target ? 12.0 * (double)n_polyak * (polyak_flag ? 0.5 : 1.0) : 0.0;
  RLREP_LAUNCHED_W("adam_polyak", s, 28.0 * (double)n + polyak, 0.0);
}

void launch_polyak(const float* p, float* target, size_t n, float tau, const int* polyak_flag, cudaStream_t s) {
  RLREP_CHECK(n % 4 == 0, "optimizer arenas are padded to float4");
  polyak_kernel<<<grid_for(n / 4, 256, 16), 256, 0, s>>>(reinterpret_cast<const float4*>(p),
                                                        reinterpret_cast<float4*>(target), n / 4, tau, polyak_flag);
  RLREP_LAUNCHED_W("polyak", s, 12.0 * (double)n * (polyak_flag ? 0.5 : 1.0), 0.0);
}

}
```

rlrep_b200/csrc/kernels.cuh:

```cuda
#pragma once
#include <cuda_runtime.h>

#include <cstdint>

#include "epilogue.cuh"

namespace rlrep {

constexpr int kMaxFeatureSteps = 16;
constexpr int kNumMetrics = 32;

struct AdamHyper {
  float step_size;
  float bc2_sqrt;
};

struct Control {
  int steps;
  int polyak_critic;
  long long t_feat, t_critic, t_actor, t_alpha;
  AdamHyper feat[kMaxFeatureSteps];
  AdamHyper critic, actor;
  double alpha_step_size, alpha_bc2_sqrt;
  double log_alpha, la_m, la_v;
  float alpha;
};

struct TickParams {
  int k_feat;
  int period;
  double lr_feat, lr_critic, lr_actor, lr_alpha;
  int critic_steps;
};

void launch_tick(Control* c, const TickParams& p, cudaStream_t s);

void launch_gather(const float* ring, int rec4, const long long* idx, int B, float* out, cudaStream_t s);
void launch_ring_write(float* ring, int rec4, long long capacity, long long start, const float* rows, int n,
                       cudaStream_t s);

void launch_ce_rows(float* logits, int ld, int rows, int cols, int diag_off, float inv_batch, float* loss_rows,
                    cudaStream_t s);

void launch_rowdot(const float* X, int ld, int rows, int D, const float* w, const float* b, float* y, cudaStream_t s);
struct RowDotJob {
  const float* X;
  const float* w;
  const float* b;
  float* y;
  int ld, D;
};
void launch_rowdot_pair(const RowDotJob& a, const RowDotJob& b, int rows, cudaStream_t s);
void launch_colreduce(const float* X, int ld, int rows, int cols, const float* u, float* out, int accumulate,
                      cudaStream_t s);
void launch_kgroup_finish(const float* ws, int groups, int M, int N, int ldw, size_t group_stride, float* C, int ldc,
                          const Epilogue& epi, cudaStream_t s);
void launch_colsum_finish(const float* partial, int chunks, int cols, float* out, cudaStream_t s);
void launch_colsum_tall(const float* X, int ld, long long rows, int cols, float* partial, int chunks, float* out,
                        cudaStream_t s);
struct ColJob {
  const float* X;
  const float* u;
  float* out;
  int ld, rows, cols;
};
constexpr int kMaxColJobs = 8;
void launch_colreduce_multi(const ColJob* jobs, int n_jobs, cudaStream_t s);
void launch_outer_dact(const float* u, const float* w, int rows, int cols, const float* aux, int ld_aux, int dact,
                       float* out, int ld_out, cudaStream_t s);

void launch_feature_loss_finalize(const float* loss_rows, int rows, const float* pred, const float* reward, int ld_r,
                                  float inv_batch, float* dpred, float* metrics , cudaStream_t s);

void launch_actor_sample(const float* head, int ld_head, int B, int A, const float* eps, float* action, int lda,
                         float* logp, cudaStream_t s, const float* obs = nullptr, int ld_obs = 0, int S = 0);
void launch_contrastive_head(float* logits, int ld, int rows, int cols, int diag_off, float inv_batch, const float* z, int ldz,
                             int D, const float* theta_w, const float* theta_b, const float* reward, int ld_r,
                             float* loss_rows, float* pred, float* dpred, float* metrics, unsigned* counter,
                             cudaStream_t s);
void launch_actor_act(const float* in, int rows, int S, int A, int H, const float* W0, int ld0, const float* b0,
                      const float* W1, int ld1, const float* b1, const float* W2, int ld2, const float* b2, int explore,
                      float* out, cudaStream_t s);
void launch_actor_sample_bwd(const float* head, int ld_head, int B, int A, const float* eps, const float* d_action,
                             int ldd, const float* dlogp_scalar, float* dhead, int ld_dhead, cudaStream_t s);

void launch_td_critic_loss(const float* reward, const float* done, int ld_rd, const float* nq1, const float* nq2,
                           const float* logp2, const float* q1, const float* q2, int B, float gamma, const Control* c,
                           float* dq1, float* dq2, float* metrics, cudaStream_t s, int norm_B = 0);

struct CriticHeadArgs {
  const float *hid_t, *hid;
  int ldh, H, B;
  const float *w2t, *b2t, *w5t, *b5t, *w2, *b2, *w5, *b5;
  const float *reward, *done;
  int ld_rd;
  const float* logp2;
  float gamma;
  const Control* c;
  float *nq1, *nq2, *q1, *q2, *dq1, *dq2, *dhid;
  int ld_dh;
  float* metrics;
  unsigned* counter;
};
void launch_critic_td_head(const CriticHeadArgs& a, cudaStream_t s);
struct ActorHeadArgs {
  const float* hid;
  int ldh, H, B;
  const float *w2, *b2, *w5, *b5;
  const float* logp;
  float target_entropy;
  int learn_alpha;
  Control* c;
  float *q1, *q2, *dq1, *dq2, *dhid;
  int ld_dh;
  float* dlogp_scalar;
  float* metrics;
  unsigned* counter;
};
void launch_actor_head(const ActorHeadArgs& a, cudaStream_t s);

void launch_actor_alpha_loss(const float* q1, const float* q2, const float* logp, int B, float target_entropy,
                             int learn_alpha, Control* c, float* dq1, float* dq2, float* dlogp_scalar, float* metrics,
                             cudaStream_t s);

void launch_actor_loss_partial(const float* q1, const float* q2, const float* logp, int B, int norm_B,
                               float target_entropy, const Control* c, float* dq1, float* dq2, float* dlogp_scalar,
                               float* partial, cudaStream_t s);
void launch_alpha_step(const float* reduced, int learn_alpha, Control* c, float* metrics, cudaStream_t s);
// ... 96 lines not shown
```

rlrep_b200/csrc/ptx.cuh:

```cuda
#pragma once
#include <cstdint>
#include <cuda.h>
#include <cuda_runtime.h>

namespace rlrep {
namespace ptx {

__device__ __forceinline__ uint32_t smem_u32(const void* p) {
  return static_cast<uint32_t>(__cvta_generic_to_shared(p));
}

__device__ __forceinline__ bool elect_one() {
  uint32_t pred = 0;
  asm volatile(
      "{\n"
      ".reg .b32 rx;\n"
      ".reg .pred px;\n"
      "elect.sync rx|px, 0xffffffff;\n"
      "selp.u32 %0, 1, 0, px;\n"
      "}\n"
      : "=r"(pred));
  return pred != 0;
}

__device__ __forceinline__ void mbar_init(uint64_t* bar, uint32_t count) {
  asm volatile("mbarrier.init.shared::cta.b64 [%0], %1;" ::"r"(smem_u32(bar)), "r"(count) : "memory");
}
__device__ __forceinline__ void fence_mbar_init() {
  asm volatile("fence.mbarrier_init.release.cluster;" ::: "memory");
}
__device__ __forceinline__ void fence_proxy_async_smem() {
  asm volatile("fence.proxy.async.shared::cta;" ::: "memory");
}
__device__ __forceinline__ void mbar_arrive_expect_tx(uint64_t* bar, uint32_t bytes) {
  asm volatile("mbarrier.arrive.expect_tx.shared::cta.b64 _, [%0], %1;" ::"r"(smem_u32(bar)), "r"(bytes)
               : "memory");
}
__device__ __forceinline__ void mbar_arrive(uint64_t* bar) {
  asm volatile("mbarrier.arrive.shared::cta.b64 _, [%0];" ::"r"(smem_u32(bar)) : "memory");
}
__device__ __forceinline__ bool mbar_try_wait(uint64_t* bar, uint32_t parity) {
  uint32_t ok;
  asm volatile(
      "{\n"
      ".reg .pred p;\n"
      "mbarrier.try_wait.parity.shared::cta.b64 p, [%1], %2;\n"
      "selp.u32 %0, 1, 0, p;\n"
      "}\n"
      : "=r"(ok)
      : "r"(smem_u32(bar)), "r"(parity)
      : "memory");
  return ok != 0;
}
__device__ __forceinline__ void mbar_wait(uint64_t* bar, uint32_t parity) {
  if (mbar_try_wait(bar, parity)) return;
  const long long t0 = clock64();
  while (!mbar_try_wait(bar, parity)) {
    if (clock64() - t0 > 4000000000LL) {
      printf("rlrep: mbarrier wait timed out (block %d,%d,%d thread %d)\n", blockIdx.x, blockIdx.y,
             blockIdx.z, threadIdx.x);
      __trap();
    }
  }
}

__device__ __forceinline__ void prefetch_tensormap(const CUtensorMap* m) {
  asm volatile("prefetch.tensormap [%0];" ::"l"(reinterpret_cast<uint64_t>(m)) : "memory");
}
__device__ __forceinline__ void tma_load_2d(void* smem_dst, const CUtensorMap* m, uint64_t* bar, int c_inner,
                                            int c_outer) {
  asm volatile(
      "cp.async.bulk.tensor.2d.shared::cluster.global.mbarrier::complete_tx::bytes [%0], [%1, {%3, %4}], [%2];"
      ::"r"(smem_u32(smem_dst)),
      "l"(reinterpret_cast<uint64_t>(m)), "r"(smem_u32(bar)), "r"(c_inner), "r"(c_outer)
      : "memory");
}
// ... 136 lines not shown
```

rlrep_b200/csrc/runtime.cu:

```cuda
#include <algorithm>
#include <atomic>

#include "agent.cuh"

namespace rlrep {

namespace {
thread_local long long g_launches = 0;
thread_local bool g_profiling = false;
thread_local std::vector<cudaEvent_t> g_events;
thread_local std::vector<const char*> g_names;
thread_local std::vector<double> g_bytes, g_flops;
}

long long launch_count() { return g_launches; }

void note_launch(const char* name, cudaStream_t stream, double bytes, double flops) {
  if (std::strncmp(name, "nccl_", 5) != 0) ++g_launches;
  if (g_profiling) {
    cudaEvent_t e;
    if (cudaEventCreate(&e) == cudaSuccess) {
      cudaEventRecord(e, stream);
      g_events.push_back(e);
      g_names.push_back(name);
// ... 289 lines not shown
    g.run(a, s);
  } else {
    GemmArgs a;
    a.M = l.out; a.N = k1; a.K = rows;
    a.A = dy.p; a.lda = dy.ld; a.a_mn = true;
    a.B = x.p; a.ldb = x.ld; a.b_mn = true;
    a.C = l.dW; a.ldc = l.ld;
    g.run(a, s);
    GemmArgs b = a;
    b.N = l.in - k1;
    b.B = x2.p; b.ldb = x2.ld;
    b.C = l.dW + k1;
    g.run(b, s);
  }
  if (bias_grad) launch_colreduce(dy.p, dy.ld, rows, l.out, nullptr, l.db, 0, s);
}

void GraphReplay::reset() {
  if (exec_) cudaGraphExecDestroy(exec_);
  if (graph_) cudaGraphDestroy(graph_);
  exec_ = nullptr;
  graph_ = nullptr;
  calls_ = 0;
}

void GraphReplay::run(cudaStream_t s, bool enabled, const std::function<void()>& body) {
  if (!enabled) {
    body();
    return;
  }
  if (exec_ != nullptr) {
    RLREP_CUDA(cudaGraphLaunch(exec_, s));
    return;
  }
  if (calls_ == 0) {
    ++calls_;
    body();
    return;
  }
  RLREP_CUDA(cudaStreamBeginCapture(s, cudaStreamCaptureModeThreadLocal));
  try {
    body();
  } catch (...) {
    cudaGraph_t g = nullptr;
    cudaStreamEndCapture(s, &g);
    if (g) cudaGraphDestroy(g);
    throw;
  }
  RLREP_CUDA(cudaStreamEndCapture(s, &graph_));
  RLREP_CUDA(cudaGraphInstantiate(&exec_, graph_, 0));
  RLREP_CUDA(cudaGraphLaunch(exec_, s));
}

}
```

Baseline: 1274.

## Enable programmatic dependent launch across kernels and merge actor sample launches

Launches most kernels, including the TF32 GEMM and chained GEMM kernels, with the programmatic stream serialization attribute. Each kernel gets griddepcontrol wait/launch_dependents calls so the next kernel's prologue (barrier init, TMEM alloc) can overlap the tail of the previous one. The two actor sample launches are merged into one two-job kernel, and in ctrlsac the actor trunk GEMMs move into the preceding feature GEMM chain. A graph-stats API is added to count kernel nodes and programmatic edges. Risks are races if a kernel reads predecessor output before its wait point, and the extra cost of the wait in tiny kernels.

```diff
diff --git a/include/rlrep_b200.h b/include/rlrep_b200.h
--- a/include/rlrep_b200.h
+++ b/include/rlrep_b200.h
@@ -261,6 +261,7 @@
 RLREP_EXPORT int rlrep_agent_act_batch(rlrep_agent* agent, const float* states_host, const float* eps_host, int rows,
                                        float* actions_host);
 RLREP_EXPORT int rlrep_agent_last_launches(rlrep_agent* agent, int* launches);
+RLREP_EXPORT int rlrep_agent_graph_stats(rlrep_agent* agent, int* kernel_nodes, int* programmatic_edges);
 
 #ifdef __cplusplus
 }
diff --git a/rlrep_b200/_lib.py b/rlrep_b200/_lib.py
--- a/rlrep_b200/_lib.py
+++ b/rlrep_b200/_lib.py
@@ -167,6 +167,7 @@
         "rlrep_pixring_gather": [vp, vp, i, vp, C.c_float, vp, vp, vp, vp, vp, vp],
         "rlrep_agent_act_batch": [vp, vp, vp, i, vp],
         "rlrep_agent_last_launches": [vp, C.POINTER(i)],
+        "rlrep_agent_graph_stats": [vp, C.POINTER(i), C.POINTER(i)],
         "rlrep_agent_train_resident": [vp, vp, vp, vp, i, C.POINTER(C.c_float)],
         "rlrep_agent_profile_train": [vp, vp, vp, vp, i, C.POINTER(C.c_char_p), C.POINTER(C.c_float),
                                       C.POINTER(C.c_double), C.POINTER(C.c_double), C.POINTER(i)],
diff --git a/rlrep_b200/agents.py b/rlrep_b200/agents.py
--- a/rlrep_b200/agents.py
+++ b/rlrep_b200/agents.py
@@ -128,6 +128,12 @@
         _lib.check(self.lib.rlrep_agent_last_launches(self.h, C.byref(v)))
         return v.value
 
+    @property
+    def graph_stats(self) -> tuple[int, int]:
+        k, p = C.c_int(), C.c_int()
+        _lib.check(self.lib.rlrep_agent_graph_stats(self.h, C.byref(k), C.byref(p)))
+        return k.value, p.value
+
 
 class SACAgent:
 
diff --git a/rlrep_b200/csrc/agent.cuh b/rlrep_b200/csrc/agent.cuh
--- a/rlrep_b200/csrc/agent.cuh
+++ b/rlrep_b200/csrc/agent.cuh
@@ -235,6 +235,7 @@
   void reset();
   void run(cudaStream_t s, bool enabled, const std::function<void()>& body);
   bool captured() const { return exec_ != nullptr; }
+  bool stats(int* kernel_nodes, int* programmatic_edges) const;
 
  private:
   int calls_ = 0;
@@ -272,6 +273,7 @@
   virtual void act(const float* state_host, const float* eps_host, float* action_host) = 0;
   virtual void act_batch(const float* states_host, const float* eps_host, int rows, float* actions_host) = 0;
   virtual void sync_targets_from_params() = 0;
+  virtual bool graph_stats(int* kernel_nodes, int* programmatic_edges) const = 0;
 
   AgentConfig cfg;
   cudaStream_t stream = nullptr;
diff --git a/rlrep_b200/csrc/agent_base.cuh b/rlrep_b200/csrc/agent_base.cuh
--- a/rlrep_b200/csrc/agent_base.cuh
+++ b/rlrep_b200/csrc/agent_base.cuh
@@ -105,6 +105,10 @@
     }
     serial_ = false;
     return profile_end(stream);
+  }
+
+  bool graph_stats(int* kernel_nodes, int* programmatic_edges) const override {
+    return graph_.stats(kernel_nodes, programmatic_edges);
   }
 
   void act(const float* state_host, const float* eps_host, float* action_host) override {
@@ -259,9 +263,10 @@
     linear_fwd(gemm_, s, B_, Mat{h1, AH_}, l1, ACT_ELU, h2, AH_);
     linear_fwd(gemm_, s, B_, Mat{h2, AH_}, l2, ACT_NONE, hd, LDH_);
   }
-  Mat actor_sample_cat(Mat obs, const float* eps, float* cat_buf, float* logp_out, int set, cudaStream_t s) {
-    launch_actor_sample(set == 0 ? head_ : bhead_, LDH_, B_, A_, eps, cat_buf + S_, LDSA_, logp_out, s, obs.p, obs.ld, S_);
-    return Mat{cat_buf, LDSA_};
+  void actor_sample_cat_pair(Mat next_obs, const float* eps_next, float* logp_next, Mat obs, const float* eps_pi,
+                             cudaStream_t s) {
+    launch_actor_sample_pair(ActorSampleJob{bhead_, eps_next, cat_next_ + S_, logp_next, next_obs.p, next_obs.ld},
+                             ActorSampleJob{head_, eps_pi, cat_pi_ + S_, logp_, obs.p, obs.ld}, LDH_, B_, A_, LDSA_, S_, s);
   }
   void actor_backward_chained(Mat obs, const float* eps) {
     const Linear l0 = a0_.view(actor_g_), l1 = a1_.view(actor_g_), l2 = a2_.view(actor_g_);
diff --git a/rlrep_b200/csrc/agent_ctrlsac.cu b/rlrep_b200/csrc/agent_ctrlsac.cu
--- a/rlrep_b200/csrc/agent_ctrlsac.cu
+++ b/rlrep_b200/csrc/agent_ctrlsac.cu
@@ -237,6 +237,10 @@
       a.C = logits_; a.ldc = B_;
       gemm_.run(a, s0);
     }
+    if (k == K_ - 1) {
+      actor_trunk(s2(), 1, s0);
+      actor_trunk(Mat{batch_, R_}, 0, s0);
+    }
     gemm_.end_chain();
     launch_contrastive_head(logits_, B_, B_, B_, 0, inv_b, zphi_, D_, D_, th.W, th.b, reward(), R_, loss_rows_, rpred_, drp_,
                             metrics_dev_ + 0, head_ctr_, s0);
@@ -289,12 +293,8 @@
     const float* eps_pi = eps_dev_ + (size_t)B_ * A_;
     const Linear l14t = c14_.view(crit_g_, true), l14 = c14_.view(crit_g_), l2 = c2_.view(crit_g_), l5 = c5_.view(crit_g_);
     const Linear l2t = c2_.view(crit_g_, true), l5t = c5_.view(crit_g_, true);
-    gemm_.begin_chain(s0);
-    actor_trunk(s2(), 1, s0);
-    actor_trunk(Mat{batch_, R_}, 0, s0);
-    gemm_.end_chain();
-    const Mat s2a = actor_sample_cat(s2(), eps_next, cat_next_, logp2_, 1, s0);
-    const Mat spi = actor_sample_cat(Mat{batch_, R_}, eps_pi, cat_pi_, logp_, 0, s0);
+    actor_sample_cat_pair(s2(), eps_next, logp2_, Mat{batch_, R_}, eps_pi, s0);
+    const Mat s2a{cat_next_, LDSA_}, spi{cat_pi_, LDSA_};
     gemm_.begin_chain(s0);
     phi_forward(s0, s2a, Mat(), 0, zmu_, h1_, h2_);
     linear_fwd(gemm_, s0, B_, Mat{zmu_, D_}, l14t, ACT_ELU, hid_t_, 2 * H_);
diff --git a/rlrep_b200/csrc/agent_vlsac.cu b/rlrep_b200/csrc/agent_vlsac.cu
--- a/rlrep_b200/csrc/agent_vlsac.cu
+++ b/rlrep_b200/csrc/agent_vlsac.cu
@@ -289,8 +289,8 @@
     actor_trunk(s2(), 1, s0);
     actor_trunk(Mat{batch_, R_}, 0, s0);
     gemm_.end_chain();
-    const Mat s2a = actor_sample_cat(s2(), eps, cat_next_, logp2_, 1, s0);
-    const Mat spi = actor_sample_cat(Mat{batch_, R_}, eps + (size_t)B_ * A_, cat_pi_, logp_, 0, s0);
+    actor_sample_cat_pair(s2(), eps, logp2_, Mat{batch_, R_}, eps + (size_t)B_ * A_, s0);
+    const Mat s2a{cat_next_, LDSA_}, spi{cat_pi_, LDSA_};
     gemm_.begin_chain(s0);
     prior_forward(s0, tgt, s2a, Mat(), 0, ph1_[0], ph2_[0], phead_[0]);
     prior_forward(s0, tgt, sa(), Mat(), 0, ph1_[1], ph2_[1], phead_[1]);
diff --git a/rlrep_b200/csrc/capi.cu b/rlrep_b200/csrc/capi.cu
--- a/rlrep_b200/csrc/capi.cu
+++ b/rlrep_b200/csrc/capi.cu
@@ -1204,6 +1204,13 @@
   *launches = agent->impl->last_launches;
   RLREP_API_END
 }
+int rlrep_agent_graph_stats(rlrep_agent* agent, int* kernel_nodes, int* programmatic_edges) {
+  RLREP_API_BEGIN_ON(agent)
+  RLREP_CHECK(agent && kernel_nodes && programmatic_edges, "null argument");
+  RLREP_CHECK(agent->impl->graph_stats(kernel_nodes, programmatic_edges),
+              "no captured graph yet (train() captures it on its second call, with use_graph on)");
+  RLREP_API_END
+}
 int rlrep_agent_train_resident(rlrep_agent* agent, rlrep_ring* ring, const int64_t* idx_host, const float* eps_host,
                                int n_steps, float* total_ms) {
   RLREP_API_BEGIN_ON(agent)
diff --git a/rlrep_b200/csrc/common.cuh b/rlrep_b200/csrc/common.cuh
--- a/rlrep_b200/csrc/common.cuh
+++ b/rlrep_b200/csrc/common.cuh
@@ -5,6 +5,7 @@
 #include <cstdio>
 #include <stdexcept>
 #include <string>
+#include <utility>
 #include <vector>
 
 namespace rlrep {
@@ -48,6 +49,25 @@
     ::rlrep::note_launch(name, stream, (bytes), (flops));       \
   } while (0)
 
+inline cudaLaunchAttribute pdl_attribute() {
+  cudaLaunchAttribute a = {};
+  a.id = cudaLaunchAttributeProgrammaticStreamSerialization;
+  a.val.programmaticStreamSerializationAllowed = 1;
+  return a;
+}
+template <typename... KernelArgs, typename... Args>
+void launch_pdl(void (*kernel)(KernelArgs...), dim3 grid, dim3 block, size_t smem, cudaStream_t stream, Args&&... args) {
+  cudaLaunchConfig_t cfg = {};
+  cfg.gridDim = grid;
+  cfg.blockDim = block;
+  cfg.dynamicSmemBytes = smem;
+  cfg.stream = stream;
+  cudaLaunchAttribute attr[1] = {pdl_attribute()};
+  cfg.attrs = attr;
+  cfg.numAttrs = 1;
+  RLREP_CUDA(cudaLaunchKernelEx(&cfg, kernel, std::forward<Args>(args)...));
+}
+
 void profile_begin(cudaStream_t stream);
 struct ProfileEntry {
   const char* name;
diff --git a/rlrep_b200/csrc/gemm_chain.cu b/rlrep_b200/csrc/gemm_chain.cu
--- a/rlrep_b200/csrc/gemm_chain.cu
+++ b/rlrep_b200/csrc/gemm_chain.cu
@@ -206,6 +206,7 @@
   __syncthreads();
   ptx::tc_fence_after_sync();
   const uint32_t tmem_base = *tmem_slot;
+  ptx::pdl_wait();
 
   if (warp == 0) {
     if (lane == 0) {
@@ -466,6 +467,7 @@
       if (lane == 0) ptx::mbar_arrive(&acc_empty[acc]);
     }
   }
+  ptx::pdl_launch_dependents();
   ptx::tc_fence_before_sync();
   __syncthreads();
   if (warp == 1) ptx::tmem_dealloc(tmem_base, 2 * kMaxBn);
@@ -761,11 +763,12 @@
   cfg.blockDim = dim3(kThreads);
   cfg.dynamicSmemBytes = kSmemBytes;
   cfg.stream = stream;
-  cudaLaunchAttribute attr[1];
+  cudaLaunchAttribute attr[2];
   attr[0].id = cudaLaunchAttributeCooperative;
   attr[0].val.cooperative = 1;
+  attr[1] = pdl_attribute();
   cfg.attrs = attr;
-  cfg.numAttrs = 1;
+  cfg.numAttrs = 2;
   RLREP_CUDA(cudaLaunchKernelEx(&cfg, gemm_chain_kernel, (const ChainGemmDesc*)d_gemms_, (const ChainTask*)d_tasks_,
                                 (const int*)d_task_begin_, d_done_, d_exit_, (int)seq_.size(), g_chain_dbg));
   RLREP_LAUNCHED_W("gemm_chain", stream, bytes_, flops_);
diff --git a/rlrep_b200/csrc/gemm_tc_kernel.cuh b/rlrep_b200/csrc/gemm_tc_kernel.cuh
--- a/rlrep_b200/csrc/gemm_tc_kernel.cuh
+++ b/rlrep_b200/csrc/gemm_tc_kernel.cuh
@@ -309,12 +309,14 @@
     }
     ptx::mbar_init(accum_bar, 1);
     ptx::fence_mbar_init();
-    for (int it = 0; it < first_round; ++it) produce(it);
   }
   if (warp == 2) {
     ptx::tmem_alloc(tmem_slot, TMEM_COLS);
     ptx::tmem_relinquish();
   }
+  ptx::pdl_wait();
+  if (warp == 0 && lane == 0)
+    for (int it = 0; it < first_round; ++it) produce(it);
   ptx::tc_fence_before_sync();
   __syncthreads();
   ptx::tc_fence_after_sync();
@@ -396,6 +398,7 @@
   if (splits > 1) ptx::cluster_sync(); else __syncthreads();
   if (threadIdx.x == 0) trace(6);
   if (warp == 2) ptx::tmem_dealloc(tmem_base, TMEM_COLS);
+  ptx::pdl_launch_dependents();
 
   {
     TileStore t;
@@ -903,9 +906,11 @@
   RLREP_CHECK(p.stages >= (p.push ? 2 : min_stages(BN)) && p.stages <= num_stages(BN), "bad pipeline depth");
   RLREP_CHECK(!p.push || (p.split_k > 1 && smem_bytes(BN, p.stages, true) <= kMaxSmem), "bad push-mode plan");
   cudaLaunchConfig_t cfg;
-  cudaLaunchAttribute attr[1];
+  cudaLaunchAttribute attr[2];
   fill_launch_config<BN, A_MN, B_MN>(cfg, attr, dim3(ceil_div(a.N, BN), ceil_div(a.M, BM), p.split_k * p.k_groups),
                                      p.split_k, p.stages, p.push, stream);
+  attr[1] = pdl_attribute();
+  cfg.numAttrs = 2;
   RLREP_CUDA(cudaLaunchKernelEx(&cfg, gemm_tf32_kernel<BN, A_MN, B_MN>, p.tmA, p.tmB, a.C, a.ldc, a.M, a.N, a.K,
                                 p.kb_per_split, p.stages,
                                 (p.push ? 1 : 0) | ((p.k_groups - 1) << 8),
diff --git a/rlrep_b200/csrc/kernels.cu b/rlrep_b200/csrc/kernels.cu
--- a/rlrep_b200/csrc/kernels.cu
+++ b/rlrep_b200/csrc/kernels.cu
@@ -3,6 +3,7 @@
 #include "common.cuh"
 #include "epilogue.cuh"
 #include "kernels.cuh"
+#include "ptx.cuh"
 #include "reduce.cuh"
 
 namespace rlrep {
@@ -19,6 +20,8 @@
 }
 
 __global__ void tick_kernel(Control* c, const TickParams p) {
+  ptx::pdl_wait();
+  ptx::pdl_launch_dependents();
   const int lane = threadIdx.x;
   if (blockIdx.x != 0 || lane >= 32) return;
   const long long t_feat = c->t_feat, t_critic = c->t_critic, t_actor = c->t_actor, t_alpha = c->t_alpha;
@@ -44,6 +47,8 @@
 
 __global__ void gather_kernel(const float4* __restrict__ ring, int rec4, const long long* __restrict__ idx, int B,
                               float4* __restrict__ out) {
+  ptx::pdl_wait();
+  ptx::pdl_launch_dependents();
   const int total = B * rec4;
   for (int i = blockIdx.x * blockDim.x + threadIdx.x; i < total; i += gridDim.x * blockDim.x) {
     const int b = i / rec4, c = i - b * rec4;
@@ -213,6 +218,8 @@
 };
 __global__ void __launch_bounds__(1024) colreduce_multi_kernel(const ColJobs jobs) {
   __shared__ float part[32][33];
+  ptx::pdl_wait();
+  ptx::pdl_launch_dependents();
   const ColJob& jb = jobs.j[blockIdx.y];
   const int tx = threadIdx.x & 31, ty = threadIdx.x >> 5;
   const int j = blockIdx.x * 32 + tx;
@@ -296,6 +303,8 @@
                                                                unsigned* __restrict__ counter, int rows) {
   __shared__ float scratch[33];
   __shared__ bool last;
+  ptx::pdl_wait();
+  ptx::pdl_launch_dependents();
   const int row = blockIdx.x;
   float* l = logits + (size_t)row * ld;
   float mx = -INFINITY;
@@ -359,9 +368,19 @@
 
 constexpr float kLogStdMin = -5.f, kLogStdMax = 2.f;
 
-__global__ void actor_sample_kernel(const float* __restrict__ head, int ld_head, int B, int A,
-                                    const float* __restrict__ eps, float* __restrict__ action, int lda,
-                                    float* __restrict__ logp, const float* __restrict__ obs, int ld_obs, int S) {
+struct ActorSampleJobs {
+  ActorSampleJob j[2];
+};
+__global__ void actor_sample_kernel(const ActorSampleJobs jobs, int ld_head, int B, int A, int lda, int S) {
+  ptx::pdl_wait();
+  ptx::pdl_launch_dependents();
+  const ActorSampleJob& jb = jobs.j[blockIdx.y];
+  const float* __restrict__ head = jb.head;
+  const float* __restrict__ eps = jb.eps;
+  float* __restrict__ action = jb.action;
+  float* __restrict__ logp = jb.logp;
+  const float* __restrict__ obs = jb.obs;
+  const int ld_obs = jb.ld_obs;
   const int b = (blockIdx.x * blockDim.x + threadIdx.x) >> 5, lane = threadIdx.x & 31;
   if (b >= B) return;
   const float* h = head + (size_t)b * ld_head;
@@ -432,6 +451,8 @@
 __global__ void actor_sample_bwd_kernel(const float* __restrict__ head, int ld_head, int B, int A,
                                         const float* __restrict__ eps, const float* __restrict__ d_action, int ldd,
                                         const float* __restrict__ dlogp_scalar, float* __restrict__ dhead, int ld_dh) {
+  ptx::pdl_wait();
+  ptx::pdl_launch_dependents();
   const int i = blockIdx.x * blockDim.x + threadIdx.x;
   if (i >= B * A) return;
   const int b = i / A, j = i - b * A;
@@ -556,6 +577,8 @@
   __shared__ float scratch[33];
   __shared__ float bc[2];
   __shared__ bool last;
+  ptx::pdl_wait();
+  ptx::pdl_launch_dependents();
   const int row = blockIdx.x, tid = threadIdx.x, H = a.H;
   const float* ht = a.hid_t + (size_t)row * a.ldh;
   const float* h = a.hid + (size_t)row * a.ldh;
@@ -613,6 +636,8 @@
   __shared__ float scratch[33];
   __shared__ float bc[2];
   __shared__ bool last;
+  ptx::pdl_wait();
+  ptx::pdl_launch_dependents();
   const int row = blockIdx.x, tid = threadIdx.x, H = a.H;
   const float* h = a.hid + (size_t)row * a.ldh;
   float q1 = block_sum<256>(head_dot(h, a.w2, H, tid), scratch);
@@ -723,6 +748,8 @@
                                                           const AdamHyper* __restrict__ hyper,
                                                           float4* __restrict__ target, size_t n4_polyak, float tau,
                                                           const int* __restrict__ polyak_flag) {
+  ptx::pdl_wait();
+  ptx::pdl_launch_dependents();
   const float ss = hyper->step_size, bc2s = hyper->bc2_sqrt;
   const bool do_polyak = target != nullptr && (polyak_flag == nullptr || *polyak_flag != 0);
   const float omt = 1.f - tau;
@@ -979,13 +1006,13 @@
 
 void launch_tick(Control* c, const TickParams& p, cudaStream_t s) {
   RLREP_CHECK(p.k_feat <= kMaxFeatureSteps, "too many feature steps per update");
-  tick_kernel<<<1, 32, 0, s>>>(c, p);
+  launch_pdl(tick_kernel, 1, 32, 0, s, c, p);
   RLREP_LAUNCHED("tick", s);
 }
 
 void launch_gather(const float* ring, int rec4, const long long* idx, int B, float* out, cudaStream_t s) {
-  gather_kernel<<<grid_for((size_t)B * rec4, 256), 256, 0, s>>>(reinterpret_cast<const float4*>(ring), rec4, idx, B,
-                                                               reinterpret_cast<float4*>(out));
+  launch_pdl(gather_kernel, grid_for((size_t)B * rec4, 256), 256, 0, s, reinterpret_cast<const float4*>(ring), rec4, idx, B,
+             reinterpret_cast<float4*>(out));
   RLREP_LAUNCHED_W("gather", s, 2.0 * 16.0 * (double)B * rec4, 0.0);
 }
 
@@ -1056,7 +1083,7 @@
     js.j[i] = jobs[i];
     if (jobs[i].cols > max_cols) max_cols = jobs[i].cols;
   }
-  colreduce_multi_kernel<<<dim3(ceil_div(max_cols, 32), n_jobs), 1024, 0, s>>>(js);
+  launch_pdl(colreduce_multi_kernel, dim3(ceil_div(max_cols, 32), n_jobs), 1024, 0, s, js);
   RLREP_LAUNCHED("colreduce_multi", s);
 }
 
@@ -1077,23 +1104,34 @@
                              int D, const float* theta_w, const float* theta_b, const float* reward, int ld_r,
                              float* loss_rows, float* pred, float* dpred, float* metrics, unsigned* counter,
                              cudaStream_t s) {
-  contrastive_head_kernel<<<rows, 256, 0, s>>>(logits, ld, cols, diag_off, inv_batch, z, ldz, D, theta_w, theta_b, reward, ld_r,
-                                               loss_rows, pred, dpred, metrics, counter, rows);
+  launch_pdl(contrastive_head_kernel, rows, 256, 0, s, logits, ld, cols, diag_off, inv_batch, z, ldz, D, theta_w, theta_b,
+             reward, ld_r, loss_rows, pred, dpred, metrics, counter, rows);
   RLREP_LAUNCHED_W("contrastive_head", s, 3.0 * 4.0 * (double)rows * cols + 4.0 * (double)rows * D, 0.0);
 }
 
 void launch_critic_td_head(const CriticHeadArgs& a, cudaStream_t s) {
-  critic_td_head_kernel<<<a.B, 256, 0, s>>>(a);
+  launch_pdl(critic_td_head_kernel, a.B, 256, 0, s, a);
   RLREP_LAUNCHED_W("critic_td_head", s, 4.0 * a.B * (4.0 * a.H + 2.0 * a.H), 0.0);
 }
 void launch_actor_head(const ActorHeadArgs& a, cudaStream_t s) {
-  actor_head_kernel<<<a.B, 256, 0, s>>>(a);
+  launch_pdl(actor_head_kernel, a.B, 256, 0, s, a);
   RLREP_LAUNCHED_W("actor_head", s, 4.0 * a.B * (4.0 * a.H), 0.0);
 }
 
 void launch_actor_sample(const float* head, int ld_head, int B, int A, const float* eps, float* action, int lda,
                          float* logp, cudaStream_t s, const float* obs, int ld_obs, int S) {
-  actor_sample_kernel<<<ceil_div(B * 32, 128), 128, 0, s>>>(head, ld_head, B, A, eps, action, lda, logp, obs, ld_obs, S);
+  ActorSampleJobs js;
+  js.j[0] = ActorSampleJob{head, eps, action, logp, obs, ld_obs};
+  js.j[1] = js.j[0];
+  launch_pdl(actor_sample_kernel, dim3(ceil_div(B * 32, 128), 1), 128, 0, s, js, ld_head, B, A, lda, S);
+  RLREP_LAUNCHED("actor_sample", s);
+}
+void launch_actor_sample_pair(const ActorSampleJob& j0, const ActorSampleJob& j1, int ld_head, int B, int A, int lda, int S,
+                              cudaStream_t s) {
+  ActorSampleJobs js;
+  js.j[0] = j0;
+  js.j[1] = j1;
+  launch_pdl(actor_sample_kernel, dim3(ceil_div(B * 32, 128), 2), 128, 0, s, js, ld_head, B, A, lda, S);
   RLREP_LAUNCHED("actor_sample", s);
 }
 
@@ -1108,8 +1146,8 @@
 
 void launch_actor_sample_bwd(const float* head, int ld_head, int B, int A, const float* eps, const float* d_action,
                              int ldd, const float* dlogp_scalar, float* dhead, int ld_dhead, cudaStream_t s) {
-  actor_sample_bwd_kernel<<<ceil_div(B * A, 128), 128, 0, s>>>(head, ld_head, B, A, eps, d_action, ldd, dlogp_scalar,
-                                                               dhead, ld_dhead);
+  launch_pdl(actor_sample_bwd_kernel, ceil_div(B * A, 128), 128, 0, s, head, ld_head, B, A, eps, d_action, ldd, dlogp_scalar,
+             dhead, ld_dhead);
   RLREP_LAUNCHED("actor_sample_bwd", s);
 }
 
@@ -1203,9 +1241,9 @@
                         size_t n_polyak, float tau, const int* polyak_flag, cudaStream_t s) {
   RLREP_CHECK(n % 4 == 0 && n_polyak % 4 == 0, "optimizer arenas are padded to float4");
   const size_t n4 = n / 4;
-  adam_polyak_kernel<<<grid_for(n4, 256, 16), 256, 0, s>>>(
-      reinterpret_cast<float4*>(p), reinterpret_cast<const float4*>(g), reinterpret_cast<float4*>(m),
-      reinterpret_cast<float4*>(v), n4, hyper, reinterpret_cast<float4*>(target), n_polyak / 4, tau, polyak_flag);
+  launch_pdl(adam_polyak_kernel, grid_for(n4, 256, 16), 256, 0, s, reinterpret_cast<float4*>(p),
+             reinterpret_cast<const float4*>(g), reinterpret_cast<float4*>(m), reinterpret_cast<float4*>(v), n4, hyper,
+             reinterpret_cast<float4*>(target), n_polyak / 4, tau, polyak_flag);
   const double polyak = target ? 12.0 * (double)n_polyak * (polyak_flag ? 0.5 : 1.0) : 0.0;
   RLREP_LAUNCHED_W("adam_polyak", s, 28.0 * (double)n + polyak, 0.0);
 }
diff --git a/rlrep_b200/csrc/kernels.cuh b/rlrep_b200/csrc/kernels.cuh
--- a/rlrep_b200/csrc/kernels.cuh
+++ b/rlrep_b200/csrc/kernels.cuh
@@ -74,6 +74,16 @@
 
 void launch_actor_sample(const float* head, int ld_head, int B, int A, const float* eps, float* action, int lda,
                          float* logp, cudaStream_t s, const float* obs = nullptr, int ld_obs = 0, int S = 0);
+struct ActorSampleJob {
+  const float* head;
+  const float* eps;
+  float* action;
+  float* logp;
+  const float* obs;
+  int ld_obs;
+};
+void launch_actor_sample_pair(const ActorSampleJob& j0, const ActorSampleJob& j1, int ld_head, int B, int A, int lda, int S,
+                              cudaStream_t s);
 void launch_contrastive_head(float* logits, int ld, int rows, int cols, int diag_off, float inv_batch, const float* z, int ldz,
                              int D, const float* theta_w, const float* theta_b, const float* reward, int ld_r,
                              float* loss_rows, float* pred, float* dpred, float* metrics, unsigned* counter,
diff --git a/rlrep_b200/csrc/ptx.cuh b/rlrep_b200/csrc/ptx.cuh
--- a/rlrep_b200/csrc/ptx.cuh
+++ b/rlrep_b200/csrc/ptx.cuh
@@ -22,6 +22,9 @@
       : "=r"(pred));
   return pred != 0;
 }
+
+__device__ __forceinline__ void pdl_wait() { asm volatile("griddepcontrol.wait;" ::: "memory"); }
+__device__ __forceinline__ void pdl_launch_dependents() { asm volatile("griddepcontrol.launch_dependents;" ::: "memory"); }
 
 __device__ __forceinline__ void mbar_init(uint64_t* bar, uint32_t count) {
   asm volatile("mbarrier.init.shared::cta.b64 [%0], %1;" ::"r"(smem_u32(bar)), "r"(count) : "memory");
diff --git a/rlrep_b200/csrc/runtime.cu b/rlrep_b200/csrc/runtime.cu
--- a/rlrep_b200/csrc/runtime.cu
+++ b/rlrep_b200/csrc/runtime.cu
@@ -365,4 +365,29 @@
   RLREP_CUDA(cudaGraphLaunch(exec_, s));
 }
 
-}
+bool GraphReplay::stats(int* kernel_nodes, int* programmatic_edges) const {
+  if (exec_ == nullptr) return false;
+  size_t n_nodes = 0;
+  RLREP_CUDA(cudaGraphGetNodes(graph_, nullptr, &n_nodes));
+  std::vector<cudaGraphNode_t> nodes(n_nodes);
+  RLREP_CUDA(cudaGraphGetNodes(graph_, nodes.data(), &n_nodes));
+  int kernels = 0;
+  for (cudaGraphNode_t n : nodes) {
+    cudaGraphNodeType t;
+    RLREP_CUDA(cudaGraphNodeGetType(n, &t));
+    if (t == cudaGraphNodeTypeKernel) ++kernels;
+  }
+  size_t n_edges = 0;
+  RLREP_CUDA(cudaGraphGetEdges_v2(graph_, nullptr, nullptr, nullptr, &n_edges));
+  std::vector<cudaGraphNode_t> from(n_edges), to(n_edges);
+  std::vector<cudaGraphEdgeData> data(n_edges);
+  RLREP_CUDA(cudaGraphGetEdges_v2(graph_, from.data(), to.data(), data.data(), &n_edges));
+  int programmatic = 0;
+  for (size_t i = 0; i < n_edges; ++i)
+    if (data[i].type == cudaGraphDependencyTypeProgrammatic) ++programmatic;
+  *kernel_nodes = kernels;
+  *programmatic_edges = programmatic;
+  return true;
+}
+
+}
```

Result: faster. 1334 (median of 6 runs) (+4.7%).
